# Siverteh/semantic-slam-master

Hardware: NVIDIA B200
Metric: frame-pairs/sec extract+match @640x480, 2048 kpts (higher is better)
Workload: dtype f16x3 (fp32 in/out)

## Files before the change

include/sslam_b200.h:

```cpp
#ifndef SSLAM_B200_H_
#define SSLAM_B200_H_

#include <stddef.h>
#include <stdint.h>

#ifdef __cplusplus
extern "C" {
#endif

#define SSLAM_ABI_VERSION 4

enum {
  SSLAM_OK = 0,
  SSLAM_EINVAL = -1,
  SSLAM_EUNSUPPORTED = -2,
  SSLAM_EWORKSPACE = -3,
  SSLAM_ECUDA = -4,
  SSLAM_ENODEVICE = -5,
  SSLAM_ERANGE = -6
};

enum {
  SSLAM_INFO_BRANCH = 0,
  SSLAM_INFO_NCAND = 1,
  SSLAM_INFO_TIES = 2,
  SSLAM_INFO_NLOCALMAX = 3
};

enum {
  SSLAM_SIM_F32 = 0,
  SSLAM_SIM_TF32X3 = 1,
  SSLAM_SIM_BF16 = 2,
  SSLAM_SIM_F16X3 = 3
};

enum {
  SSLAM_MATCH_M1 = 1,
  SSLAM_MATCH_M2 = 2,
  SSLAM_MATCH_M3 = 3,
  SSLAM_MATCH_M4 = 4,
  SSLAM_MATCH_M5 = 5
};

int sslam_abi_version(void);

int sslam_last_error(char* buf, size_t len);

int sslam_device_check(void);

uint64_t sslam_launch_count(void);

int sslam_profile_enable(int on);
int sslam_profile_kinds(void);
const char* sslam_profile_kind_name(int kind);
int sslam_profile_read(int kind, double* total_ms, uint64_t* launches);

size_t sslam_decode_workspace_bytes(int B, int H, int W, int K);
int sslam_decode_topk_f32(const float* sal, int from_logits, int B, int H, int W, int K,
                          int nms_radius, float pct, float floor, float* kpts_xy, float* scores,
                          int32_t* info, void* ws, size_t ws_bytes, void* stream);

int sslam_nms_f32(const float* sal, int B, int H, int W, int nms_radius, float* out, void* stream);

int sslam_gather_bilinear_f32(const float* feat, const float* kpts, int B, int h, int w, int C,
                              int N, int coords, float* out, void* out_hi, void* out_lo,
                              void* stream);

int sslam_l2norm_rows(const float* in, int rows, int D, float eps, float* out_f32,
                      void* out_bf16, void* out_hi, void* out_lo, void* stream);

size_t sslam_refiner_packed_bytes(int C, int Hd, int D, int blocks);
int sslam_refiner_pack_weights(const float* const* params, int C, int Hd, int D, int blocks,
                               void* packed, size_t packed_bytes, void* stream);
size_t sslam_refiner_workspace_bytes(int rows, int C, int Hd, int D, int blocks);
int sslam_refiner_forward_f32(const float* const* params, const void* packed, const float* x,
                              const void* x_hi, const void* x_lo,
                              int rows, int C, int Hd, int D, int blocks, float eps_norm,
                              float* out_f32, void* out_bf16, void* out_hi, void* out_lo,
                              void* ws, size_t ws_bytes, void* stream);
int sslam_refiner_range_check(void* stream);

size_t sslam_match_workspace_bytes(int F1, int F2, int P, int N, int M, int D, int dtype);
int sslam_match_top2(const void* bank1, const void* bank1_lo, int F1, const void* bank2,
                     const void* bank2_lo, int F2, const int32_t* pair_index, int dtype,
                     int P, int N, int M, int D, int32_t* nn12, float* best12, float* second12,
                     int32_t* nn21, float* best21, void* ws, size_t ws_bytes, void* stream);

int sslam_match_finalize(int variant, const double* params ,
                         const int32_t* pair_index, int P, int N, int M, const int32_t* nn12,
                         const float* best12, const float* second12, const int32_t* nn21,
                         const float* best21, const float* scores1, const float* scores2,
                         const float* inten1, const float* inten2, int32_t* pairs,
                         float* pair_scores, int32_t* counts, void* stream);

int sslam_nn_points(const float* kpts1, int F1, const float* kpts2, int F2, const double* H,
                    const int32_t* pair_index, int P, int N, int M, void* min_dist, int32_t* argmin,
                    void* stream);

int sslam_gt_matches(const void* min_dist, const int32_t* argmin, int is_double, double threshold, int P,
                     int N, int32_t* pairs, int32_t* counts, void* stream);

int sslam_eval_matches(const int32_t* pred, const int32_t* pred_counts, int pred_stride,
                       const int32_t* gt, const int32_t* gt_counts, int gt_stride, int P, int N,
                       int32_t* scratch, int32_t* out, void* stream);

size_t sslam_ransac_workspace_bytes(int P, int L, int iters);
int sslam_ransac_homography(const float* kpts1, int F1, const float* kpts2, int F2,
                            const int32_t* pair_index, int P, int N, int M,
                            const int32_t* pairs, const float* pair_scores, const int32_t* counts, int L,
                            int iters, double threshold, uint64_t seed,
                            double* H, int32_t* out_pairs, float* out_scores,
                            int32_t* out_counts, uint8_t* inlier_mask,
                            void* ws, size_t ws_bytes, void* stream);

int sslam_heatmap_from_cells_f32(const float* logits, int B, int Hc, int Wc, int cell, int border,
                                 float* heat, void* stream);

size_t sslam_selector_packed_bytes(int C, int hidden);
int sslam_selector_pack_weights(const float* conv1_weight, int C, int hidden, void* packed,
                                size_t packed_bytes, void* stream);
size_t sslam_selector_workspace_bytes(int B, int H, int W, int C);
int sslam_selector_head_f32(const float* feat, const void* packed, const float* conv1_bias,
                            const float* conv2_weight, const float* conv2_bias, int B, int H, int W,
                            int C, int hidden, int apply_sigmoid, float* out, void* ws,
                            size_t ws_bytes, void* stream);

#ifdef __cplusplus
}
#endif
#endif
```

semantic-slam-master_b200/csrc/gather.cu:

```cuda
#include <cuda_bf16.h>
#include <cuda_fp16.h>

#include "common.cuh"

namespace sslam {
namespace {

constexpr int WARPS_PER_BLOCK = 8;

struct Taps {
  int off[4];
  float w[4];
};

struct TapGeom {
  int xi0, yi0;
  bool vx0, vx1, vy0, vy1;
  float w[4];
};

__device__ __forceinline__ TapGeom tap_geometry(float x, float y, int H, int W, int coords) {
  if (coords == 1) {
    x = __fmul_rn(__fsub_rn(x, 8.0f), 0.0625f);
    y = __fmul_rn(__fsub_rn(y, 8.0f), 0.0625f);
  }
  const float wm1 = (float)(W - 1), hm1 = (float)(H - 1);
  float nx = __fsub_rn(__fdiv_rn(__fmul_rn(2.0f, x), wm1), 1.0f);
  float ny = __fsub_rn(__fdiv_rn(__fmul_rn(2.0f, y), hm1), 1.0f);
  float ix = __fmul_rn(__fmul_rn(__fadd_rn(nx, 1.0f), 0.5f), wm1);
  float iy = __fmul_rn(__fmul_rn(__fadd_rn(ny, 1.0f), 0.5f), hm1);
  float x0 = floorf(ix), y0 = floorf(iy);
  float x1 = __fadd_rn(x0, 1.0f), y1 = __fadd_rn(y0, 1.0f);
  float wx0 = __fsub_rn(x1, ix), wx1 = __fsub_rn(ix, x0);
  float wy0 = __fsub_rn(y1, iy), wy1 = __fsub_rn(iy, y0);
  TapGeom g;
  g.w[0] = __fmul_rn(wx0, wy0); g.w[1] = __fmul_rn(wx1, wy0);
  g.w[2] = __fmul_rn(wx0, wy1); g.w[3] = __fmul_rn(wx1, wy1);
  g.xi0 = (int)x0; g.yi0 = (int)y0;
  const int xi1 = (int)x1, yi1 = (int)y1;
  g.vx0 = (x0 >= 0.f) && (g.xi0 < W); g.vx1 = (x1 >= 0.f) && (xi1 < W);
  g.vy0 = (y0 >= 0.f) && (g.yi0 < H); g.vy1 = (y1 >= 0.f) && (yi1 < H);
  return g;
}

__device__ __forceinline__ Taps make_taps(float x, float y, int H, int W, int C, int coords) {
  const TapGeom g = tap_geometry(x, y, H, W, coords);
  Taps t;
#pragma unroll
  for (int i = 0; i < 4; ++i) t.w[i] = g.w[i];
  const int xi1 = g.xi0 + 1, yi1 = g.yi0 + 1;
  t.off[0] = (g.vx0 && g.vy0) ? (g.yi0 * W + g.xi0) * C : -1;
  t.off[1] = (g.vx1 && g.vy0) ? (g.yi0 * W + xi1) * C : -1;
  t.off[2] = (g.vx0 && g.vy1) ? (yi1 * W + g.xi0) * C : -1;
  t.off[3] = (g.vx1 && g.vy1) ? (yi1 * W + xi1) * C : -1;
  return t;
}

__device__ __forceinline__ float blend(float a, float b, float c, float d, const Taps& t) {
  float acc = __fmul_rn(a, t.w[0]);
  acc = __fmaf_rn(b, t.w[1], acc);
  acc = __fmaf_rn(c, t.w[2], acc);
  acc = __fmaf_rn(d, t.w[3], acc);
  return acc;
}

template <bool VEC4>
__global__ void __launch_bounds__(WARPS_PER_BLOCK * 32)
gather_kernel(const float* __restrict__ feat, const float* __restrict__ kpts, int B, int H, int W,
              int C, int N, int coords, float* __restrict__ out, __half* __restrict__ out_hi,
              __half* __restrict__ out_lo) {
  const int lane = threadIdx.x & 31;
  const long long kp = (long long)blockIdx.x * WARPS_PER_BLOCK + (threadIdx.x >> 5);
  if (kp >= (long long)B * N) return;
  const int b = (int)(kp / N);
  const float x = __ldg(kpts + 2 * kp), y = __ldg(kpts + 2 * kp + 1);
  const Taps t = make_taps(x, y, H, W, C, coords);
  const float* img = feat + (size_t)b * H * W * C;
  float* o = out + (size_t)kp * C;
  if (VEC4) {
    const float4 zero = make_float4(0.f, 0.f, 0.f, 0.f);
    for (int c = lane * 4; c < C; c += 128) {
      float4 v0 = t.off[0] >= 0 ? __ldg(reinterpret_cast<const float4*>(img + t.off[0] + c)) : zero;
      float4 v1 = t.off[1] >= 0 ? __ldg(reinterpret_cast<const float4*>(img + t.off[1] + c)) : zero;
      float4 v2 = t.off[2] >= 0 ? __ldg(reinterpret_cast<const float4*>(img + t.off[2] + c)) : zero;
      float4 v3 = t.off[3] >= 0 ? __ldg(reinterpret_cast<const float4*>(img + t.off[3] + c)) : zero;
      float4 r;
      r.x = blend(v0.x, v1.x, v2.x, v3.x, t);
      r.y = blend(v0.y, v1.y, v2.y, v3.y, t);
      r.z = blend(v0.z, v1.z, v2.z, v3.z, t);
      r.w = blend(v0.w, v1.w, v2.w, v3.w, t);
      if (out) *reinterpret_cast<float4*>(o + c) = r;
      if (out_hi) {
        __half h4[4], l4[4];
        const float rr[4] = {r.x, r.y, r.z, r.w};
#pragma unroll
        for (int i = 0; i < 4; ++i) {
          h4[i] = __float2half_rn(rr[i]);
          l4[i] = __float2half_rn(__fmul_rn(__fsub_rn(rr[i], __half2float(h4[i])), 2048.0f));
        }
        *reinterpret_cast<uint2*>(out_hi + (size_t)kp * C + c) = *reinterpret_cast<uint2*>(h4);
        *reinterpret_cast<uint2*>(out_lo + (size_t)kp * C + c) = *reinterpret_cast<uint2*>(l4);
      }
    }
  } else {
    for (int c = lane; c < C; c += 32) {
      float v0 = t.off[0] >= 0 ? __ldg(img + t.off[0] + c) : 0.f;
      float v1 = t.off[1] >= 0 ? __ldg(img + t.off[1] + c) : 0.f;
      float v2 = t.off[2] >= 0 ? __ldg(img + t.off[2] + c) : 0.f;
      float v3 = t.off[3] >= 0 ? __ldg(img + t.off[3] + c) : 0.f;
      const float r = blend(v0, v1, v2, v3, t);
      if (out) o[c] = r;
      if (out_hi) {
        const __half h = __float2half_rn(r);
        out_hi[(size_t)kp * C + c] = h;
        out_lo[(size_t)kp * C + c] = __float2half_rn(__fmul_rn(__fsub_rn(r, __half2float(h)), 2048.0f));
      }
    }
  }
}

constexpr int BAND_THREADS = 512;

__device__ __forceinline__ uint32_t smem_addr_u32(const void* p) {
  return static_cast<uint32_t>(__cvta_generic_to_shared(p));
}
__device__ __forceinline__ void band_bar_wait(uint64_t* bar, uint32_t parity) {
  const uint32_t addr = smem_addr_u32(bar);
  uint32_t ok = 0;
  while (!ok)
    asm volatile(
        "{\n"
        ".reg .pred p;\n"
        "mbarrier.try_wait.parity.shared::cta.b64 p, [%1], %2;\n"
        "selp.u32 %0, 1, 0, p;\n"
        "}\n"
        : "=r"(ok)
        : "r"(addr), "r"(parity)
        : "memory");
}

struct __align__(4) BandGeo { float w[4]; short xi0; short band; };

template <bool PAIR>
__global__ void __launch_bounds__(BAND_THREADS, 1)
gather_band_kernel(const float* __restrict__ feat, const float* __restrict__ kpts, int B, int H, int W, int C,
                   int N, int coords, float* __restrict__ out, __half* __restrict__ out_hi,
                   __half* __restrict__ out_lo, int bands_per_group, int ngroups) {
  extern __shared__ __align__(128) unsigned char gsm[];
  const int row_bytes = W * C * 4, row_floats = W * C;
  const float* ring = reinterpret_cast<const float*>(gsm);
  BandGeo* geo = reinterpret_cast<BandGeo*>(gsm + 3 * row_bytes);
  unsigned short* list = reinterpret_cast<unsigned short*>(geo + N);
  uint64_t* bars = reinterpret_cast<uint64_t*>((reinterpret_cast<uintptr_t>(list + N) + 7) & ~(uintptr_t)7);
  __shared__ int list_n[2];
  const int tid = threadIdx.x, lane = tid & 31, warp = tid >> 5;
  const int b = blockIdx.x / ngroups, g = blockIdx.x - b * ngroups;
  const int band_lo = g * bands_per_group - 1;
  const int band_hi = min(band_lo + bands_per_group, H);
  const float* img = feat + (size_t)b * H * W * C;
  const float* kp_b = kpts + (size_t)b * N * 2;

  if (tid == 0) {
    for (int i = 0; i < 3; ++i)
      asm volatile("mbarrier.init.shared::cta.b64 [%0], 1;" ::"r"(smem_addr_u32(&bars[i])) : "memory");
    asm volatile("fence.mbarrier_init.release.cluster;" ::: "memory");
    list_n[0] = 0; list_n[1] = 0;
  }
  const int first_row = max(band_lo, 0);
  const int last_row = min(band_hi, H - 1);
  __syncthreads();
  auto issue_row = [&](int y) {
    const int slot = y % 3;
    const uint32_t bar = smem_addr_u32(&bars[slot]);
    const int use = (y - first_row) / 3;
    if (use > 0) band_bar_wait(&bars[slot], (uint32_t)(use - 1) & 1u);
    asm volatile("mbarrier.arrive.expect_tx.shared::cta.b64 _, [%0], %1;" ::"r"(bar), "r"((uint32_t)row_bytes) : "memory");
    asm volatile("cp.async.bulk.shared::cluster.global.mbarrier::complete_tx::bytes [%0], [%1], %2, [%3];" ::"r"(
                     smem_addr_u32(gsm + (size_t)slot * row_bytes)),
                 "l"(img + (size_t)y * W * C), "r"((uint32_t)row_bytes), "r"(bar)
                 : "memory");
  };
  if (tid == 0) {
    if (first_row <= last_row) issue_row(first_row);
    if (first_row + 1 <= last_row) issue_row(first_row + 1);
  }
  for (int i = tid; i < N; i += BAND_THREADS) {
    const float2 xy = __ldg(reinterpret_cast<const float2*>(kp_b) + i);
    const TapGeom t = tap_geometry(xy.x, xy.y, H, W, coords);
    BandGeo gg;
#pragma unroll
    for (int k = 0; k < 4; ++k) gg.w[k] = t.w[k];
    const bool any_x = t.vx0 || t.vx1, any_y = t.vy0 || t.vy1;
    gg.xi0 = (short)((any_x && any_y) ? (t.vx0 ? t.xi0 : -1) : -2);
    gg.band = (short)((any_x && any_y && t.vy0) ? t.yi0 : -1);
    geo[i] = gg;
  }
  __syncthreads();

  int it = 0;
  for (int y0 = band_lo; y0 < band_hi; ++y0, ++it) {
    if (tid == 0 && y0 + 2 <= last_row && y0 + 2 >= first_row + 2) issue_row(y0 + 2);
    const bool r0_ok = y0 >= 0 && y0 < H, r1_ok = y0 + 1 >= 0 && y0 + 1 < H;
    const int o0 = ((y0 + 3) % 3) * row_floats, o1 = ((y0 + 1) % 3) * row_floats;
    int* cnt = &list_n[it & 1];
    for (int i = tid; i < N; i += BAND_THREADS)
      if (geo[i].band == y0) list[atomicAdd(cnt, 1)] = (unsigned short)i;
    __syncthreads();
    const int n = *cnt;
    if (tid == 0) list_n[(it + 1) & 1] = 0;
    if (r0_ok) band_bar_wait(&bars[y0 % 3], (uint32_t)((y0 - first_row) / 3) & 1u);
    if (r1_ok) band_bar_wait(&bars[(y0 + 1) % 3], (uint32_t)((y0 + 1 - first_row) / 3) & 1u);
    for (int e = warp; e < n; e += BAND_THREADS / 32) {
      const int i = list[e];
      const BandGeo gg = geo[i];
      const size_t kp = (size_t)b * N + i;
      Taps w4;
#pragma unroll
      for (int k = 0; k < 4; ++k) w4.w[k] = gg.w[k];
      const int xi0 = gg.xi0;
      const bool vx0 = xi0 >= 0 && xi0 < W, vx1 = xi0 >= -1 && xi0 + 1 < W;
      const int t0 = (vx0 && r0_ok) ? o0 + xi0 * C : -1, t1 = (vx1 && r0_ok) ? o0 + (xi0 + 1) * C : -1;
      const int t2 = (vx0 && r1_ok) ? o1 + xi0 * C : -1, t3 = (vx1 && r1_ok) ? o1 + (xi0 + 1) * C : -1;
      const float4 zero = make_float4(0.f, 0.f, 0.f, 0.f);
      for (int c = lane * 4; c < C; c += 128) {
        const float4 a0 = t0 >= 0 ? *reinterpret_cast<const float4*>(ring + t0 + c) : zero;
        const float4 a1 = t1 >= 0 ? *reinterpret_cast<const float4*>(ring + t1 + c) : zero;
        const float4 a2 = t2 >= 0 ? *reinterpret_cast<const float4*>(ring + t2 + c) : zero;
        const float4 a3 = t3 >= 0 ? *reinterpret_cast<const float4*>(ring + t3 + c) : zero;
        float4 r;
        r.x = blend(a0.x, a1.x, a2.x, a3.x, w4);
        r.y = blend(a0.y, a1.y, a2.y, a3.y, w4);
        r.z = blend(a0.z, a1.z, a2.z, a3.z, w4);
        r.w = blend(a0.w, a1.w, a2.w, a3.w, w4);
        if (!PAIR) {
          *reinterpret_cast<float4*>(out + kp * C + c) = r;
        } else {
          const __half2 h01 = __floats2half2_rn(r.x, r.y), h23 = __floats2half2_rn(r.z, r.w);
          const float2 f01 = __half22float2(h01), f23 = __half22float2(h23);
          const __half2 l01 = __floats2half2_rn(__fmul_rn(__fsub_rn(r.x, f01.x), 2048.0f),
                                                __fmul_rn(__fsub_rn(r.y, f01.y), 2048.0f));
          const __half2 l23 = __floats2half2_rn(__fmul_rn(__fsub_rn(r.z, f23.x), 2048.0f),
                                                __fmul_rn(__fsub_rn(r.w, f23.y), 2048.0f));
          uint2 hv, lv;
          hv.x = *reinterpret_cast<const unsigned*>(&h01); hv.y = *reinterpret_cast<const unsigned*>(&h23);
          lv.x = *reinterpret_cast<const unsigned*>(&l01); lv.y = *reinterpret_cast<const unsigned*>(&l23);
          *reinterpret_cast<uint2*>(out_hi + kp * C + c) = hv;
          *reinterpret_cast<uint2*>(out_lo + kp * C + c) = lv;
        }
      }
    }
    __syncthreads();
  }
}

template <bool VEC4>
__global__ void __launch_bounds__(WARPS_PER_BLOCK * 32)
l2norm_kernel(const float* __restrict__ in, int rows, int D, float eps, float* __restrict__ out_f32,
              __nv_bfloat16* __restrict__ out_bf16, __half* __restrict__ out_hi, __half* __restrict__ out_lo) {
  const int lane = threadIdx.x & 31;
  const long long row = (long long)blockIdx.x * WARPS_PER_BLOCK + (threadIdx.x >> 5);
  if (row >= rows) return;
  const float* src = in + (size_t)row * D;
  float ss = 0.f;
  if (VEC4) {
    for (int c = lane * 4; c < D; c += 128) {
      float4 v = __ldg(reinterpret_cast<const float4*>(src + c));
      ss = __fmaf_rn(v.x, v.x, ss); ss = __fmaf_rn(v.y, v.y, ss);
      ss = __fmaf_rn(v.z, v.z, ss); ss = __fmaf_rn(v.w, v.w, ss);
    }
  } else {
    for (int c = lane; c < D; c += 32) { float v = __ldg(src + c); ss = __fmaf_rn(v, v, ss); }
  }
  ss = warp_reduce_sum(ss);
  const float denom = fmaxf(sqrtf(ss), eps);
  if (VEC4) {
    for (int c = lane * 4; c < D; c += 128) {
      float4 v = __ldg(reinterpret_cast<const float4*>(src + c));
      float4 r = make_float4(__fdiv_rn(v.x, denom), __fdiv_rn(v.y, denom), __fdiv_rn(v.z, denom),
                             __fdiv_rn(v.w, denom));
      if (out_f32) *reinterpret_cast<float4*>(out_f32 + (size_t)row * D + c) = r;
      if (out_bf16) {
        __nv_bfloat162 lo = __floats2bfloat162_rn(r.x, r.y), hi = __floats2bfloat162_rn(r.z, r.w);
        uint2 pk = make_uint2(*reinterpret_cast<unsigned*>(&lo), *reinterpret_cast<unsigned*>(&hi));
        *reinterpret_cast<uint2*>(out_bf16 + (size_t)row * D + c) = pk;
      }
      if (out_hi) {
        __half h4[4], l4[4];
        const float rr[4] = {r.x, r.y, r.z, r.w};
#pragma unroll
        for (int i = 0; i < 4; ++i) {
          h4[i] = __float2half_rn(rr[i]);
          l4[i] = __float2half_rn(__fmul_rn(__fsub_rn(rr[i], __half2float(h4[i])), 2048.0f));
        }
        *reinterpret_cast<uint2*>(out_hi + (size_t)row * D + c) = *reinterpret_cast<uint2*>(h4);
        *reinterpret_cast<uint2*>(out_lo + (size_t)row * D + c) = *reinterpret_cast<uint2*>(l4);
      }
    }
  } else {
    for (int c = lane; c < D; c += 32) {
      float r = __fdiv_rn(__ldg(src + c), denom);
      if (out_f32) out_f32[(size_t)row * D + c] = r;
      if (out_bf16) out_bf16[(size_t)row * D + c] = __float2bfloat16_rn(r);
      if (out_hi) {
        const __half h = __float2half_rn(r);
        out_hi[(size_t)row * D + c] = h;
        out_lo[(size_t)row * D + c] = __float2half_rn(__fmul_rn(__fsub_rn(r, __half2float(h)), 2048.0f));
      }
    }
  }
}

}
}

using namespace sslam;

extern "C" int sslam_gather_bilinear_f32(const float* feat, const float* kpts, int B, int h, int w,
                                         int C, int N, int coords, float* out, void* out_hi_, void* out_lo_,
                                         void* stream_) {
  __half* out_hi = static_cast<__half*>(out_hi_);
  __half* out_lo = static_cast<__half*>(out_lo_);
  int rc = check_device();
  if (rc) return rc;
  cudaStream_t stream = (cudaStream_t)stream_;
  SSLAM_REQUIRE(B >= 0 && h > 0 && w > 0 && C > 0 && N >= 0, SSLAM_EINVAL, "gather: bad size");
  SSLAM_REQUIRE(coords == 0 || coords == 1, SSLAM_EINVAL, "gather: coords must be 0 or 1");
  if (B == 0 || N == 0) return SSLAM_OK;
  SSLAM_REQUIRE(feat && kpts && (out || (out_hi && out_lo)), SSLAM_EINVAL, "gather: null pointer");
  SSLAM_REQUIRE((out_hi == nullptr) == (out_lo == nullptr), SSLAM_EINVAL, "gather: pair outputs go together");
  SSLAM_REQUIRE((long long)h * w * C < (1ll << 31), SSLAM_EUNSUPPORTED, "gather: map too large");
  const long long total = (long long)B * N;
  const unsigned blocks = (unsigned)((total + WARPS_PER_BLOCK - 1) / WARPS_PER_BLOCK);
  const bool vec = (C % 4 == 0) && ((reinterpret_cast<uintptr_t>(feat) & 15) == 0) &&
                   ((reinterpret_cast<uintptr_t>(out) & 15) == 0) &&
                   ((reinterpret_cast<uintptr_t>(out_hi) & 7) == 0) && ((reinterpret_cast<uintptr_t>(out_lo) & 7) == 0);
  const size_t band_smem = 3 * (size_t)w * C * 4 + (size_t)N * (sizeof(BandGeo) + 2) + 64;
  if (vec && ((size_t)w * C * 4) % 16 == 0 && N <= 65535 && band_smem <= 227 * 1024 - 256 &&
      (reinterpret_cast<uintptr_t>(kpts) & 7) == 0 && ((out != nullptr) != (out_hi != nullptr))) {
    static DeviceOnce once;
    if (once.first_use()) {
      SSLAM_CHECK_CUDA(cudaFuncSetAttribute(gather_band_kernel<true>, cudaFuncAttributeMaxDynamicSharedMemorySize,
                                            227 * 1024 - 256));
      SSLAM_CHECK_CUDA(cudaFuncSetAttribute(gather_band_kernel<false>, cudaFuncAttributeMaxDynamicSharedMemorySize,
                                            227 * 1024 - 256));
    }
    int ngroups = (8 * num_sms() + B - 1) / B;
    if (ngroups > (h + 1) / 3) ngroups = (h + 1) / 3;
    if (ngroups < 1) ngroups = 1;
    const int per = (h + 1 + ngroups - 1) / ngroups;
    ngroups = (h + 1 + per - 1) / per;
    SSLAM_LAUNCH(KK_GATHER, stream,
                 if (out_hi)
        gather_band_kernel<true><<<(unsigned)(B * ngroups), BAND_THREADS, band_smem, stream>>>(
            feat, kpts, B, h, w, C, N, coords, out, out_hi, out_lo, per, ngroups);
      else
        gather_band_kernel<false><<<(unsigned)(B * ngroups), BAND_THREADS, band_smem, stream>>>(
            feat, kpts, B, h, w, C, N, coords, out, out_hi, out_lo, per, ngroups));
    return SSLAM_OK;
  }
  SSLAM_LAUNCH(KK_GATHER, stream,
               if (vec)
      gather_kernel<true><<<blocks, WARPS_PER_BLOCK * 32, 0, stream>>>(feat, kpts, B, h, w, C, N,
                                                                      coords, out, out_hi, out_lo);
    else
      gather_kernel<false><<<blocks, WARPS_PER_BLOCK * 32, 0, stream>>>(feat, kpts, B, h, w, C, N,
                                                                     coords, out, out_hi, out_lo));
  return SSLAM_OK;
}

extern "C" int sslam_l2norm_rows(const float* in, int rows, int D, float eps, float* out_f32,
                                 void* out_bf16, void* out_hi_, void* out_lo_, void* stream_) {
  __half* out_hi = static_cast<__half*>(out_hi_);
  __half* out_lo = static_cast<__half*>(out_lo_);
  int rc = check_device();
  if (rc) return rc;
  cudaStream_t stream = (cudaStream_t)stream_;
  SSLAM_REQUIRE(rows >= 0 && D > 0, SSLAM_EINVAL, "l2norm: bad size");
  if (rows == 0) return SSLAM_OK;
  SSLAM_REQUIRE(in && (out_f32 || out_bf16 || out_hi), SSLAM_EINVAL, "l2norm: null pointer");
  SSLAM_REQUIRE((out_hi == nullptr) == (out_lo == nullptr), SSLAM_EINVAL, "l2norm: pair outputs go together");
  const unsigned blocks = (unsigned)((rows + WARPS_PER_BLOCK - 1) / WARPS_PER_BLOCK);
  const bool vec = (D % 4 == 0) && ((reinterpret_cast<uintptr_t>(in) & 15) == 0) &&
                   (!out_f32 || (reinterpret_cast<uintptr_t>(out_f32) & 15) == 0) &&
                   (!out_bf16 || (reinterpret_cast<uintptr_t>(out_bf16) & 7) == 0) &&
                   ((reinterpret_cast<uintptr_t>(out_hi) & 7) == 0) && ((reinterpret_cast<uintptr_t>(out_lo) & 7) == 0);
  SSLAM_LAUNCH(KK_L2NORM, stream,
               if (vec)
      l2norm_kernel<true><<<blocks, WARPS_PER_BLOCK * 32, 0, stream>>>(
          in, rows, D, eps, out_f32, reinterpret_cast<__nv_bfloat16*>(out_bf16), out_hi, out_lo);
    else
      l2norm_kernel<false><<<blocks, WARPS_PER_BLOCK * 32, 0, stream>>>(
          in, rows, D, eps, out_f32, reinterpret_cast<__nv_bfloat16*>(out_bf16), out_hi, out_lo));
  return SSLAM_OK;
}
```

semantic-slam-master_b200/csrc/match_f32.cu:

```cuda
#include "common.cuh"

namespace sslam {
namespace {

constexpr int BM = 128, BN = 128, BK = 16;
constexpr int LDS_ = BM + 4;
constexpr int THREADS = 256;
constexpr int MAX_D = 256;

struct Top2 {
  float best, second;
  int idx;
  __device__ __forceinline__ void init() {
    best = __int_as_float(0xff800000); second = best; idx = 0x7fffffff;
  }
  __device__ __forceinline__ void push(float v, int i) {
    if (v > best) { second = best; best = v; idx = i; }
    else second = fmaxf(second, v);
  }
  __device__ __forceinline__ void merge(float b2, float s2, int i2) {
    if (b2 > best || (b2 == best && i2 < idx)) { second = fmaxf(best, s2); best = b2; idx = i2; }
    else second = fmaxf(second, b2);
  }
};

struct MatchParams {
  const float* bank1;
  const float* bank2;
  const int32_t* pair_index;
  int P, N, M, D;
  int32_t* nn12;
  float* best12;
  float* second12;
  u64* colkeys;
};

__device__ __forceinline__ int row_of(int t, int i) { return (i < 4) ? t * 4 + i : 64 + t * 4 + (i - 4); }

__global__ void __launch_bounds__(THREADS, 1) match_f32_kernel(MatchParams p) {
  extern __shared__ __align__(16) float smem[];
  const int D = p.D, N = p.N, M = p.M;
  const int dpad = (D + BK - 1) / BK * BK;
  float* As = smem;
  float* Bs = As + (size_t)dpad * LDS_;
  u64* colpart = reinterpret_cast<u64*>(Bs + 2 * BK * LDS_);

  const int pair = blockIdx.y;
  int ia = pair, ib = pair;
  if (p.pair_index) { ia = p.pair_index[2 * pair]; ib = p.pair_index[2 * pair + 1]; }
  const float* A = p.bank1 + (size_t)ia * N * D;
  const float* Bm = p.bank2 + (size_t)ib * M * D;
  const int row0 = blockIdx.x * BM;
  const int tid = threadIdx.x, tx = tid & 15, ty = tid >> 4, lane = tid & 31, warp = tid >> 5;

  const int dq = dpad / 4;
  for (int e = tid; e < BM * dq; e += THREADS) {
    int r = e / dq, kq = e - r * dq;
    float4 v = make_float4(0.f, 0.f, 0.f, 0.f);
    if (row0 + r < N && kq * 4 < D) v = __ldg(reinterpret_cast<const float4*>(A + (size_t)(row0 + r) * D + kq * 4));
    As[(kq * 4 + 0) * LDS_ + r] = v.x; As[(kq * 4 + 1) * LDS_ + r] = v.y;
    As[(kq * 4 + 2) * LDS_ + r] = v.z; As[(kq * 4 + 3) * LDS_ + r] = v.w;
  }

  const int nkb = dpad / BK;
  const int ntile = (M + BN - 1) / BN;
  const int total = nkb * ntile;

  float4 stage[2];
  auto fetch = [&](int it) {
    int ct = it / nkb, kb = it - ct * nkb;
#pragma unroll
    for (int j = 0; j < 2; ++j) {
      int e = tid + THREADS * j, col = e >> 2, kq = e & 3;
      int gc = ct * BN + col, gk = kb * BK + kq * 4;
      stage[j] = (gc < M && gk < D) ? __ldg(reinterpret_cast<const float4*>(Bm + (size_t)gc * D + gk))
                                    : make_float4(0.f, 0.f, 0.f, 0.f);
    }
  };
  auto commit = [&](int buf) {
    float* dst = Bs + buf * BK * LDS_;
#pragma unroll
    for (int j = 0; j < 2; ++j) {
      int e = tid + THREADS * j, col = e >> 2, kq = e & 3;
      dst[(kq * 4 + 0) * LDS_ + col] = stage[j].x; dst[(kq * 4 + 1) * LDS_ + col] = stage[j].y;
      dst[(kq * 4 + 2) * LDS_ + col] = stage[j].z; dst[(kq * 4 + 3) * LDS_ + col] = stage[j].w;
    }
  };

  Top2 rowtop[8];
#pragma unroll
  for (int i = 0; i < 8; ++i) rowtop[i].init();
  float acc[8][8];
#pragma unroll
  for (int i = 0; i < 8; ++i)
#pragma unroll
    for (int j = 0; j < 8; ++j) acc[i][j] = 0.f;

  fetch(0);
  commit(0);
  __syncthreads();

  for (int it = 0; it < total; ++it) {
    const int buf = it & 1;
    const int ct = it / nkb, kb = it - ct * nkb;
    if (it + 1 < total) fetch(it + 1);
    const float* a_base = As + (size_t)(kb * BK) * LDS_;
    const float* b_base = Bs + buf * BK * LDS_;
#pragma unroll
    for (int kk = 0; kk < BK; ++kk) {
      float4 a0 = *reinterpret_cast<const float4*>(a_base + kk * LDS_ + ty * 4);
      float4 a1 = *reinterpret_cast<const float4*>(a_base + kk * LDS_ + 64 + ty * 4);
      float4 b0 = *reinterpret_cast<const float4*>(b_base + kk * LDS_ + tx * 4);
      float4 b1 = *reinterpret_cast<const float4*>(b_base + kk * LDS_ + 64 + tx * 4);
      float a[8] = {a0.x, a0.y, a0.z, a0.w, a1.x, a1.y, a1.z, a1.w};
      float b[8] = {b0.x, b0.y, b0.z, b0.w, b1.x, b1.y, b1.z, b1.w};
#pragma unroll
      for (int i = 0; i < 8; ++i)
#pragma unroll
        for (int j = 0; j < 8; ++j) acc[i][j] = __fmaf_rn(a[i], b[j], acc[i][j]);
    }
    if (kb == nkb - 1) {
      const int c0 = ct * BN;
#pragma unroll
      for (int i = 0; i < 8; ++i) {
        Top2 t; t.init();
#pragma unroll
        for (int j = 0; j < 8; ++j) {
          int gc = c0 + row_of(tx, j);
          if (gc < M) t.push(acc[i][j], gc);
        }
#pragma unroll
        for (int o = 8; o > 0; o >>= 1) {
          float b2 = __shfl_xor_sync(0xffffffffu, t.best, o);
          float s2 = __shfl_xor_sync(0xffffffffu, t.second, o);
          int i2 = __shfl_xor_sync(0xffffffffu, t.idx, o);
          t.merge(b2, s2, i2);
        }
        rowtop[i].merge(t.best, t.second, t.idx);
      }
#pragma unroll
      for (int j = 0; j < 8; ++j) {
        u64 key = 0;
        float bv = 0.f; int bi = -1;
#pragma unroll
        for (int i = 0; i < 8; ++i) {
          int gr = row0 + row_of(ty, i);
          if (gr < N && (bi < 0 || acc[i][j] > bv)) { bv = acc[i][j]; bi = gr; }
        }
        if (bi >= 0) key = pack_key(bv, (u32)bi);
        u64 other = __shfl_xor_sync(0xffffffffu, key, 16);
        key = other > key ? other : key;
        if (lane < 16) colpart[warp * BN + row_of(tx, j)] = key;
      }
      __syncthreads();
      if (tid < BN) {
        u64 k = colpart[tid];
#pragma unroll
        for (int w = 1; w < 8; ++w) { u64 o = colpart[w * BN + tid]; k = o > k ? o : k; }
        if (c0 + tid < M && k) atomicMax(p.colkeys + (size_t)pair * M + c0 + tid, k);
      }
#pragma unroll
      for (int i = 0; i < 8; ++i)
#pragma unroll
        for (int j = 0; j < 8; ++j) acc[i][j] = 0.f;
    }
    if (it + 1 < total) commit(buf ^ 1);
    __syncthreads();
  }

  if (tx == 0) {
#pragma unroll
    for (int i = 0; i < 8; ++i) {
      int gr = row0 + row_of(ty, i);
      if (gr < N) {
        size_t o = (size_t)pair * N + gr;
        p.nn12[o] = rowtop[i].idx;
        p.best12[o] = rowtop[i].best;
        p.second12[o] = rowtop[i].second;
      }
    }
  }
}

__global__ void unpack_cols_kernel(const u64* __restrict__ keys, long long total, int32_t* nn21,
                                   float* best21) {
  long long i = (long long)blockIdx.x * blockDim.x + threadIdx.x;
  if (i >= total) return;
  u64 k = keys[i];
  nn21[i] = (int32_t)key_index(k);
  best21[i] = key_value(k);
}

struct FinalizeParams {
  int variant;
  float prm[8];
  double prm_d[2];
  const int32_t* pair_index;
  int P, N, M;
  const int32_t* nn12; const float* best12; const float* second12;
  const int32_t* nn21; const float* best21;
  const float* scores1; const float* scores2; const float* inten1; const float* inten2;
  int32_t* pairs; float* pair_scores; int32_t* counts;
};

__device__ __forceinline__ bool accept_row(const FinalizeParams& f, int pair, int ia, int ib, int i,
                                           int& j, float& score) {
  const size_t ro = (size_t)pair * f.N + i;
  j = f.nn12[ro];
  const float best = f.best12[ro];
  const bool mutual = (f.nn21[(size_t)pair * f.M + j] == i);
  switch (f.variant) {
    case SSLAM_MATCH_M1: {
      float second = fmaxf(f.second12[ro], -1.0f);
      score = best;
      if (f.prm[1] != 0.f) return mutual && ((double)best > __dmul_rn((double)second, f.prm_d[0]));
      return mutual && (best > __fmul_rn(second, f.prm[0]));
    }
    case SSLAM_MATCH_M2: {
      float s1 = f.scores1[(size_t)ia * f.N + i], s2 = f.scores2[(size_t)ib * f.M + j];
      float avg = __fdiv_rn(__fadd_rn(s1, s2), 2.0f);
      bool ok = mutual && (avg >= f.prm[1]) && (best >= f.prm[2]);
      if (f.inten1 && f.inten2) {
        float a = f.inten1[(size_t)ia * f.N + i], b = f.inten2[(size_t)ib * f.M + j];
        ok = ok && (__fdiv_rn(__fadd_rn(a, b), 2.0f) >= f.prm[3]);
      }
      score = __fadd_rn(__fmul_rn(f.prm[4], best), __fmul_rn(f.prm[0], avg));
      return ok;
    }
    case SSLAM_MATCH_M3: {
      float ratio = __fdiv_rn(f.second12[ro], __fadd_rn(best, 1e-8f));
      score = __fsub_rn(1.0f, best);
      return mutual && (ratio < f.prm[0]);
    }
    case SSLAM_MATCH_M4:
      score = best;
      return mutual;
    default:
      score = best;
      return best > f.prm[0];
  }
}

__global__ void __launch_bounds__(256) finalize_kernel(FinalizeParams f) {
  __shared__ int scan[256];
  __shared__ int total_s;
  const int pair = blockIdx.x, tid = threadIdx.x;
  int ia = pair, ib = pair;
  if (f.pair_index) { ia = f.pair_index[2 * pair]; ib = f.pair_index[2 * pair + 1]; }
  const int seg = (f.N + 255) / 256;
  const int beg = min(f.N, tid * seg), end = min(f.N, beg + seg);
  int cnt = 0;
  for (int i = beg; i < end; ++i) { int j; float s; cnt += accept_row(f, pair, ia, ib, i, j, s) ? 1 : 0; }
  scan[tid] = cnt;
  __syncthreads();
  for (int o = 1; o < 256; o <<= 1) {
    int v = (tid >= o) ? scan[tid - o] : 0;
    __syncthreads();
    scan[tid] += v;
    __syncthreads();
  }
  int pos = scan[tid] - cnt;
  if (tid == 255) total_s = scan[255];
  __syncthreads();
  const int total = total_s;
  int32_t* pr = f.pairs + (size_t)pair * f.N * 2;
  float* ps = f.pair_scores + (size_t)pair * f.N;
  for (int i = beg; i < end; ++i) {
    int j; float s;
    if (accept_row(f, pair, ia, ib, i, j, s)) { pr[2 * pos] = i; pr[2 * pos + 1] = j; ps[pos] = s; ++pos; }
  }
  for (int i = total + tid; i < f.N; i += 256) { pr[2 * i] = -1; pr[2 * i + 1] = -1; ps[i] = 0.f; }
  if (tid == 0) f.counts[pair] = total;
}

}

int match_top2_tc(const void* bank1, const void* bank1_lo, int F1, const void* bank2, const void* bank2_lo,
                  int F2, const int32_t* pair_index,
                  int dtype, int P, int N, int M, int D, int32_t* nn12, float* best12, float* second12,
                  u64* colkeys, void* ws_extra, size_t ws_extra_bytes, cudaStream_t stream);
size_t match_tc_extra_workspace(int P, int N, int M, int D, int dtype, int F1, int F2);

}

using namespace sslam;

extern "C" size_t sslam_match_workspace_bytes(int F1, int F2, int P, int N, int M, int D, int dtype) {
  if (P <= 0 || N <= 0 || M <= 0) return 0;
  size_t base = align_up((size_t)P * M * sizeof(u64), 256);
  if (dtype != SSLAM_SIM_F32) base += match_tc_extra_workspace(P, N, M, D, dtype, F1, F2);
  return base;
}

extern "C" int sslam_match_top2(const void* bank1, const void* bank1_lo, int F1, const void* bank2,
                                const void* bank2_lo, int F2, const int32_t* pair_index,
                                int dtype, int P, int N, int M, int D, int32_t* nn12, float* best12,
                                float* second12, int32_t* nn21, float* best21, void* ws,
                                size_t ws_bytes, void* stream_) {
  int rc = check_device();
  if (rc) return rc;
  cudaStream_t stream = (cudaStream_t)stream_;
  SSLAM_REQUIRE(P >= 0 && N >= 0 && M >= 0 && D > 0, SSLAM_EINVAL, "match: bad size");
  if (P == 0 || N == 0) return SSLAM_OK;
  SSLAM_REQUIRE(M > 0, SSLAM_EINVAL, "match: M must be > 0 (argmax of an empty row)");
  SSLAM_REQUIRE(bank1 && bank2 && nn12 && best12 && second12 && nn21 && best21 && ws, SSLAM_EINVAL,
                "match: null pointer");
  SSLAM_REQUIRE(D % 4 == 0 && D <= MAX_D, SSLAM_EUNSUPPORTED, "match: D=%d (need D%%4==0, D<=256)", D);
  SSLAM_REQUIRE(dtype == SSLAM_SIM_F32 || dtype == SSLAM_SIM_TF32X3 || dtype == SSLAM_SIM_BF16 ||
                    dtype == SSLAM_SIM_F16X3,
                SSLAM_EINVAL, "match: unknown dtype %d", dtype);
  SSLAM_REQUIRE(F1 > 0 && F2 > 0 && (pair_index || (F1 >= P && F2 >= P)), SSLAM_EINVAL,
                "match: banks hold %d / %d sets but %d implicit pairs were requested", F1, F2, P);
  const bool presplit = bank1_lo != nullptr || bank2_lo != nullptr;
  SSLAM_REQUIRE(!presplit || (dtype == SSLAM_SIM_F16X3 && bank1_lo && bank2_lo), SSLAM_EINVAL,
                "match: pre-split banks need SSLAM_SIM_F16X3 and both lo arrays");
  {
    const size_t need = presplit ? align_up((size_t)P * M * sizeof(u64), 256)
                                 : sslam_match_workspace_bytes(F1, F2, P, N, M, D, dtype);
    SSLAM_REQUIRE(ws_bytes >= need, SSLAM_EWORKSPACE, "match: workspace %zu < %zu", ws_bytes, need);
  }
  SSLAM_REQUIRE((reinterpret_cast<uintptr_t>(bank1) & 15) == 0 &&
                (reinterpret_cast<uintptr_t>(bank2) & 15) == 0, SSLAM_EINVAL,
                "match: descriptor banks must be 16-byte aligned");
  u64* colkeys = reinterpret_cast<u64*>(ws);
  const size_t colbytes = align_up((size_t)P * M * sizeof(u64), 256);
  SSLAM_CHECK_CUDA(cudaMemsetAsync(colkeys, 0, (size_t)P * M * sizeof(u64), stream));

  if (dtype == SSLAM_SIM_F32) {
    MatchParams mp;
    mp.bank1 = (const float*)bank1; mp.bank2 = (const float*)bank2; mp.pair_index = pair_index;
    mp.P = P; mp.N = N; mp.M = M; mp.D = D;
    mp.nn12 = nn12; mp.best12 = best12; mp.second12 = second12; mp.colkeys = colkeys;
    const int dpad = (D + BK - 1) / BK * BK;
    size_t smem = ((size_t)dpad * LDS_ + 2 * BK * LDS_) * 4 + 8 * BN * sizeof(u64);
    static DeviceOnce once;
    if (once.first_use()) {
      SSLAM_CHECK_CUDA(cudaFuncSetAttribute(match_f32_kernel,
                                            cudaFuncAttributeMaxDynamicSharedMemorySize, 200 * 1024));
    }
    dim3 grid((N + BM - 1) / BM, P);
    SSLAM_LAUNCH(KK_MATCH_F32, stream,
                 match_f32_kernel<<<grid, THREADS, smem, stream>>>(mp));
  } else {
    rc = match_top2_tc(bank1, bank1_lo, F1, bank2, bank2_lo, F2, pair_index, dtype, P, N, M, D, nn12, best12,
                       second12, colkeys,
                       reinterpret_cast<char*>(ws) + colbytes, ws_bytes - colbytes, stream);
    if (rc) return rc;
  }
  const long long total = (long long)P * M;
  SSLAM_LAUNCH(KK_UNPACK, stream,
               unpack_cols_kernel<<<(unsigned)((total + 255) / 256), 256, 0, stream>>>(colkeys, total, nn21, best21));
  return SSLAM_OK;
}

extern "C" int sslam_match_finalize(int variant, const double* params, const int32_t* pair_index,
                                    int P, int N, int M, const int32_t* nn12, const float* best12,
                                    const float* second12, const int32_t* nn21, const float* best21,
                                    const float* scores1, const float* scores2, const float* inten1,
                                    const float* inten2, int32_t* pairs, float* pair_scores,
                                    int32_t* counts, void* stream_) {
  int rc = check_device();
  if (rc) return rc;
  cudaStream_t stream = (cudaStream_t)stream_;
  SSLAM_REQUIRE(variant >= SSLAM_MATCH_M1 && variant <= SSLAM_MATCH_M5, SSLAM_EINVAL,
                "finalize: unknown variant %d", variant);
  SSLAM_REQUIRE(P >= 0 && N >= 0 && M > 0, SSLAM_EINVAL, "finalize: bad size");
  if (P == 0) return SSLAM_OK;
  SSLAM_REQUIRE(params && nn12 && best12 && second12 && nn21 && best21 && pairs && pair_scores && counts,
                SSLAM_EINVAL, "finalize: null pointer");
  SSLAM_REQUIRE(variant != SSLAM_MATCH_M2 || (scores1 && scores2), SSLAM_EINVAL,
                "finalize: M2 needs saliency scores");
  FinalizeParams f;
  f.variant = variant;
  for (int i = 0; i < 8; ++i) f.prm[i] = (float)params[i];
  f.prm_d[0] = params[0]; f.prm_d[1] = params[1];
  f.pair_index = pair_index; f.P = P; f.N = N; f.M = M;
  f.nn12 = nn12; f.best12 = best12; f.second12 = second12; f.nn21 = nn21; f.best21 = best21;
  f.scores1 = scores1; f.scores2 = scores2; f.inten1 = inten1; f.inten2 = inten2;
  f.pairs = pairs; f.pair_scores = pair_scores; f.counts = counts;
  SSLAM_LAUNCH(KK_FINALIZE, stream,
               finalize_kernel<<<P, 256, 0, stream>>>(f));
  return SSLAM_OK;
}
```

semantic-slam-master_b200/csrc/match_tc.cu:

```cuda
#include "tc_common.cuh"

#include <mutex>

namespace sslam {

using namespace tc;

long long* g_match_dbg = nullptr;

namespace {

constexpr int BM = 128, BN = 128;
constexpr int BLOCK_BYTES = BM * 128;
constexpr int NUM_THREADS = 192;
constexpr int TP_LD = 36;

template <int MODE> struct Cfg;
template <> struct Cfg<SSLAM_SIM_TF32X3> {
  static constexpr int TERMS = 2, STAGES = 3, BK = 32, ACC_COLS = 2 * BN, TMEM_COLS = 512;
  static constexpr bool TF32 = true;
  static constexpr uint32_t FMT = FMT_TF32;
  static constexpr float CROSS_SCALE = 1.0f;
};
struct TcParams {
// ... 351 lines not shown
          tcgen05_fence_after();
          const uint32_t tmem_d = tmem_base + acc * C::ACC_COLS;
          for (int kb = 0; kb < nkb; ++kb) {
            if (dbg_on) tq = clock64();
            if (ct == 0) mbar_wait(&afull[kb], (uint32_t)(it & 1));
            if (dbg_on) w_afull += clock64() - tq;
            if (dbg_on) tq = clock64();
            mbar_wait(&full[stage], phase);
            if (dbg_on) w_full += clock64() - tq;
            tcgen05_fence_after();
            const uint32_t sa = smem_u32(a_res + (kb * C::TERMS) * BLOCK_BYTES);
            const uint32_t sb = smem_u32(b_stages + stage * L::B_STAGE);
            const uint64_t a_hi = make_smem_desc_sw128(sa);
            const uint64_t a_lo = make_smem_desc_sw128(sa + BLOCK_BYTES);
            const uint64_t b_hi = make_smem_desc_sw128(sb);
            const uint64_t b_lo = make_smem_desc_sw128(sb + L::B_TILE);
#pragma unroll
            for (int k = 0; k < 4; ++k) {
              const uint64_t adv = (uint64_t)(k * 32 >> 4);
              const uint32_t first = (kb | k) ? 1u : 0u;
              if (C::TERMS == 2) {
                umma_ss_pair(tmem_d + BN, a_lo + adv, b_hi + adv, idesc, first);
                umma_ss_pair(tmem_d + BN, a_hi + adv, b_lo + adv, idesc, 1u);
              }
              umma_ss_pair(tmem_d, a_hi + adv, b_hi + adv, idesc, first);
            }
            tcgen05_commit_pair(&empty[stage], 3);
            if (ct == ntile - 1) tcgen05_commit_pair(&aempty[kb], 3);
            if (kb == nkb - 1) tcgen05_commit_pair(&tfull[acc], 3);
            if (++stage == C::B_STAGES) { stage = 0; phase ^= 1; }
          }
        }
      }
      if (p.dbg) {
        long long* d = p.dbg + 4 * blockIdx.x;
        d[0] = clock64() - t_begin; d[1] = w_full; d[2] = w_tempty; d[3] = w_afull;
      }
    }
  } else {
    const int q = warp & 3;
    const int ew = warp - 2;
    const int half = ew >> 2;
    const int et = threadIdx.x - 64;
    float* tp = transp + ew * 32 * R_UNIT;
    const int sc = lane & 15, srh = lane >> 4;
    const float NEG_INF = __int_as_float(0xff800000);
    int tc = 0, it = 0;
    const uint32_t tempty_leader0 = mapa_u32(smem_u32(&tempty[0]), 0);
    const uint32_t tempty_leader1 = mapa_u32(smem_u32(&tempty[1]), 0);
    for (int item = pair_id; item < nitems; item += npairs, ++it) {
      const int pair = item / strips2;
      const int row0 = (2 * (item - pair * strips2) + (int)rank) * BM;
      const int grow = row0 + q * 32 + lane;
      const bool row_ok = grow < p.N;
      int nvalid = p.N - (row0 + q * 32);
      nvalid = nvalid < 0 ? 0 : (nvalid > 32 ? 32 : nvalid);
      float best = NEG_INF, second = NEG_INF;
      int bidx = 0x7fffffff;
      for (int ct = 0; ct < ntile; ++ct, ++tc) {
        const int acc = tc & 1;
        mbar_wait(&tfull[acc], ((uint32_t)tc >> 1) & 1u);
        tcgen05_fence_after();
        u64* cp = colpart + (acc * 4 + q) * BN;
        const int c0 = ct * BN;
        uint32_t r[R_UNIT], rs[R_UNIT];
        {
          const uint32_t taddr = tmem_base + ((uint32_t)(q * 32) << 16) + acc * C::ACC_COLS + half * 64;
          tmem_ld_32x16(taddr, r);
          if (C::TERMS == 2) tmem_ld_32x16(taddr + BN, rs);
        }
#pragma unroll
        for (int un = 0; un < 64 / R_UNIT; ++un) {
          const int col0 = half * 64 + un * R_UNIT;
          const int gc0 = c0 + col0;
          float v[R_UNIT];
          tmem_ld_wait();
#pragma unroll
          for (int j = 0; j < R_UNIT; ++j)
            v[j] = C::TERMS == 2 ? __fmaf_rn(__uint_as_float(rs[j]), C::CROSS_SCALE, __uint_as_float(r[j]))
                                 : __uint_as_float(r[j]);
          if (un + 1 < 64 / R_UNIT) {
            const uint32_t taddr = tmem_base + ((uint32_t)(q * 32) << 16) + acc * C::ACC_COLS + col0 + R_UNIT;
            tmem_ld_32x16(taddr, r);
            if (C::TERMS == 2) tmem_ld_32x16(taddr + BN, rs);
          }
          if (gc0 + R_UNIT > p.M) {
#pragma unroll
            for (int j = 0; j < R_UNIT; ++j)
              if (gc0 + j >= p.M) v[j] = NEG_INF;
          }
          {
            float tb[R_UNIT / 2], ts[R_UNIT / 2];
#pragma unroll
            for (int j = 0; j < R_UNIT / 2; ++j) {
              tb[j] = fmaxf(v[2 * j], v[2 * j + 1]);
              ts[j] = fminf(v[2 * j], v[2 * j + 1]);
            }
#pragma unroll
            for (int w = R_UNIT / 4; w >= 1; w >>= 1) {
#pragma unroll
              for (int j = 0; j < w; ++j) {
                const float lo = fminf(tb[2 * j], tb[2 * j + 1]);
                ts[j] = fmaxf(fmaxf(ts[2 * j], ts[2 * j + 1]), lo);
                tb[j] = fmaxf(tb[2 * j], tb[2 * j + 1]);
              }
            }
            const float ub = tb[0];
            second = fmaxf(fmaxf(second, ts[0]), fminf(best, ub));
            if (ub > best) {
              best = ub;
              int f = R_UNIT - 1;
#pragma unroll
              for (int j = R_UNIT - 2; j >= 0; --j) f = (v[j] == ub) ? j : f;
              bidx = gc0 + f;
            }
          }
          if (nvalid < 32 && !row_ok) {
#pragma unroll
            for (int j = 0; j < R_UNIT; ++j) v[j] = NEG_INF;
          }
          __syncwarp();
#pragma unroll
          for (int j = 0; j < R_UNIT / 4; ++j)
            *reinterpret_cast<float4*>(tp + lane * R_UNIT + ((j ^ ((lane >> 1) & 3)) << 2)) =
                make_float4(v[4 * j], v[4 * j + 1], v[4 * j + 2], v[4 * j + 3]);
          __syncwarp();
          float cv[16];
#pragma unroll
          for (int rr = 0; rr < 16; ++rr)
            cv[rr] = tp[(2 * rr + srh) * R_UNIT + ((((sc >> 2) ^ (rr & 3))) << 2) + (sc & 3)];
          float m0 = cv[0], m1 = cv[8];
          int r0 = 0, r1 = 8;
#pragma unroll
          for (int rr = 1; rr < 8; ++rr) {
            if (cv[rr] > m0) { m0 = cv[rr]; r0 = rr; }
            if (cv[8 + rr] > m1) { m1 = cv[8 + rr]; r1 = 8 + rr; }
          }
          float cm = m0;
          int cr = r0;
          if (m1 > m0) { cm = m1; cr = r1; }
          cr = 2 * cr + srh;
          {
            const float om = __shfl_xor_sync(0xffffffffu, cm, 16);
            const int orow = __shfl_xor_sync(0xffffffffu, cr, 16);
            if (om > cm || (om == cm && orow < cr)) { cm = om; cr = orow; }
          }
          if (srh == 0) cp[col0 + sc] = (nvalid > 0) ? pack_key(cm, (u32)(row0 + q * 32 + cr)) : 0ull;
        }
        tcgen05_fence_before();
        __syncwarp();
        if (lane == 0) mbar_arrive_cluster(acc ? tempty_leader1 : tempty_leader0);
        named_bar_sync(1, 32 * R_EPI_WARPS);
        if (et < BN) {
          const u64* base = colpart + acc * 4 * BN;
          u64 k = base[et];
#pragma unroll
          for (int w = 1; w < 4; ++w) { u64 o = base[w * BN + et]; k = o > k ? o : k; }
          if (c0 + et < p.M && k) atomicMax(p.colkeys + (size_t)pair * p.M + c0 + et, k);
        }
      }
      float* rm = rowmerge + (it & 1) * (BM * 3) + (q * 32 + lane) * 3;
      if (half == 1) { rm[0] = best; rm[1] = __int_as_float(bidx); rm[2] = second; }
      named_bar_sync(1, 32 * R_EPI_WARPS);
      if (half == 0 && row_ok) {
        const float ob = rm[0], os = rm[2];
        const int oi = __float_as_int(rm[1]);
        const float lo_best = fminf(best, ob);
        float sec = fmaxf(fmaxf(second, os), lo_best);
        if (ob > best || (ob == best && oi < bidx)) { best = ob; bidx = oi; }
        const size_t o = (size_t)pair * p.N + grow;
        p.nn12[o] = bidx; p.best12[o] = best; p.second12[o] = sec;
      }
    }
  }
  tcgen05_fence_before();
  cluster_sync_all();
  if (warp == 1) tmem_dealloc_pair(tmem_base, C::TMEM_COLS);
}

__global__ void split_tf32_kernel(const float4* __restrict__ src, float4* __restrict__ hi,
                                  float4* __restrict__ lo, size_t n4) {
  size_t i = (size_t)blockIdx.x * blockDim.x + threadIdx.x;
  const size_t stride = (size_t)gridDim.x * blockDim.x;
  for (; i < n4; i += stride) {
    float4 x = __ldg(src + i), h, l;
    h.x = to_tf32_rna(x.x); h.y = to_tf32_rna(x.y); h.z = to_tf32_rna(x.z); h.w = to_tf32_rna(x.w);
    l.x = to_tf32_rna(__fsub_rn(x.x, h.x)); l.y = to_tf32_rna(__fsub_rn(x.y, h.y));
    l.z = to_tf32_rna(__fsub_rn(x.z, h.z)); l.w = to_tf32_rna(__fsub_rn(x.w, h.w));
    hi[i] = h; lo[i] = l;
  }
}

__global__ void split_f16_kernel(const float4* __restrict__ src, uint2* __restrict__ hi,
                                 uint2* __restrict__ lo, size_t n4) {
  size_t i = (size_t)blockIdx.x * blockDim.x + threadIdx.x;
  const size_t stride = (size_t)gridDim.x * blockDim.x;
  for (; i < n4; i += stride) {
    const float4 x = __ldg(src + i);
    __half h[4], l[4];
    split_f16(x.x, h[0], l[0]); split_f16(x.y, h[1], l[1]);
    split_f16(x.z, h[2], l[2]); split_f16(x.w, h[3], l[3]);
    hi[i] = *reinterpret_cast<uint2*>(h);
    lo[i] = *reinterpret_cast<uint2*>(l);
  }
}

typedef CUresult (*EncodeTiledFn)(CUtensorMap*, CUtensorMapDataType, cuuint32_t, void*, const cuuint64_t*,
                                  const cuuint64_t*, const cuuint32_t*, const cuuint32_t*,
                                  CUtensorMapInterleave, CUtensorMapSwizzle, CUtensorMapL2promotion,
                                  CUtensorMapFloatOOBfill);
EncodeTiledFn g_encode = nullptr;
std::once_flag g_encode_once;

}

namespace tc {
int make_tensor_map_2d(CUtensorMap* map, const void* base, uint64_t rows, uint64_t cols,
                       uint32_t box_rows, uint32_t box_cols, int elem_bytes, int swizzle_bytes) {
  std::call_once(g_encode_once, [] {
    void* fn = nullptr;
    cudaDriverEntryPointQueryResult qres;
    if (cudaGetDriverEntryPoint("cuTensorMapEncodeTiled", &fn, cudaEnableDefault, &qres) == cudaSuccess &&
        qres == cudaDriverEntryPointSuccess)
      g_encode = reinterpret_cast<EncodeTiledFn>(fn);
  });
  SSLAM_REQUIRE(g_encode != nullptr, SSLAM_ECUDA, "cuTensorMapEncodeTiled entry point not available");
  if (swizzle_bytes < 0) return SSLAM_OK;
  cuuint64_t dims[2] = {cols, rows};
  cuuint64_t strides[1] = {cols * (uint64_t)elem_bytes};
  cuuint32_t box[2] = {box_cols, box_rows};
  cuuint32_t estr[2] = {1, 1};
  CUresult r = g_encode(map, elem_bytes == 2 ? CU_TENSOR_MAP_DATA_TYPE_BFLOAT16 : CU_TENSOR_MAP_DATA_TYPE_FLOAT32,
                        2, const_cast<void*>(base), dims, strides, box, estr, CU_TENSOR_MAP_INTERLEAVE_NONE,
                        swizzle_bytes == 128 ? CU_TENSOR_MAP_SWIZZLE_128B
                                             : swizzle_bytes == 64 ? CU_TENSOR_MAP_SWIZZLE_64B : CU_TENSOR_MAP_SWIZZLE_NONE,
                        CU_TENSOR_MAP_L2_PROMOTION_L2_256B,
                        CU_TENSOR_MAP_FLOAT_OOB_FILL_NONE);
  SSLAM_REQUIRE(r == CUDA_SUCCESS, SSLAM_ECUDA, "cuTensorMapEncodeTiled failed with CUresult %d", (int)r);
  return SSLAM_OK;
}
int make_tensor_map_nhwc(CUtensorMap* map, const void* base, uint64_t B, uint64_t H, uint64_t W, uint64_t C,
                         uint32_t box_h, uint32_t box_w, uint32_t box_c) {
  int rc = make_tensor_map_2d(nullptr, nullptr, 0, 0, 0, 0, 0, -1);
  if (rc) return rc;
  cuuint64_t dims[4] = {C, W, H, B};
  cuuint64_t strides[3] = {C * 2, W * C * 2, H * W * C * 2};
  cuuint32_t box[4] = {box_c, box_w, box_h, 1};
  cuuint32_t estr[4] = {1, 1, 1, 1};
  CUresult r = g_encode(map, CU_TENSOR_MAP_DATA_TYPE_BFLOAT16, 4, const_cast<void*>(base), dims, strides, box, estr,
                        CU_TENSOR_MAP_INTERLEAVE_NONE, CU_TENSOR_MAP_SWIZZLE_128B, CU_TENSOR_MAP_L2_PROMOTION_L2_256B,
                        CU_TENSOR_MAP_FLOAT_OOB_FILL_NONE);
  SSLAM_REQUIRE(r == CUDA_SUCCESS, SSLAM_ECUDA, "cuTensorMapEncodeTiled (NHWC) failed with CUresult %d", (int)r);
  return SSLAM_OK;
}
}

namespace {

struct BankPlan {
  bool shared;
  size_t frames_a, frames_b, off_b_frames;
};

BankPlan plan_banks(const float* b1, int F1, const float* b2, int F2, int N, int M, int D) {
  BankPlan pl{false, (size_t)F1, (size_t)F2, 0};
  if (N != M) return pl;
  const size_t frame = (size_t)N * D;
  const float* end1 = b1 + (size_t)F1 * frame;
  if (b2 >= b1 && b2 <= end1 && ((size_t)(b2 - b1) % frame) == 0) {
    pl.shared = true;
    pl.off_b_frames = (size_t)(b2 - b1) / frame;
    size_t uni = pl.off_b_frames + (size_t)F2;
    pl.frames_a = uni > (size_t)F1 ? uni : (size_t)F1;
  }
  return pl;
}

}

size_t match_tc_extra_workspace(int P, int N, int M, int D, int dtype, int F1, int F2) {
  (void)P;
  if (dtype != SSLAM_SIM_TF32X3 && dtype != SSLAM_SIM_F16X3) return 0;
  const size_t e = dtype == SSLAM_SIM_F16X3 ? 2 : 4;
  return 2 * align_up((size_t)F1 * N * D * e, 256) + 2 * align_up((size_t)F2 * M * D * e, 256) + 1024;
}

template <int MODE>
static int launch_tc(const CUtensorMap& a_hi, const CUtensorMap& a_lo, const CUtensorMap& b_hi,
                     const CUtensorMap& b_lo, const TcParams& tp, cudaStream_t stream) {
  using L = SmemLayout<MODE>;
  static DeviceOnce once;
  if (once.first_use()) {
    SSLAM_CHECK_CUDA(cudaFuncSetAttribute(match_tc_kernel<MODE>, cudaFuncAttributeMaxDynamicSharedMemorySize,
                                          L::TOTAL));
  }
  const int strips = (tp.N + BM - 1) / BM;
  SSLAM_LAUNCH(KK_MATCH_TC, stream,
               match_tc_kernel<MODE><<<strips * tp.P, NUM_THREADS, L::TOTAL, stream>>>(a_hi, a_lo, b_hi, b_lo, tp));
  return SSLAM_OK;
}

template <int MODE>
static int launch_res(const CUtensorMap& a_hi, const CUtensorMap& a_lo, const CUtensorMap& b_hi,
                      const CUtensorMap& b_lo, const TcParams& tp, cudaStream_t stream) {
  using L = RSmem<MODE>;
  static DeviceOnce once;
  if (once.first_use()) {
    SSLAM_CHECK_CUDA(cudaFuncSetAttribute(match_res_kernel<MODE>, cudaFuncAttributeMaxDynamicSharedMemorySize,
                                          L::TOTAL));
  }
  const int items = ((((tp.N + BM - 1) / BM) + 1) / 2) * tp.P;
  const int pairs = items < num_sms() / 2 ? items : num_sms() / 2;
  const int grid = 2 * pairs;
  SSLAM_LAUNCH(KK_MATCH_TC, stream,
               match_res_kernel<MODE><<<grid, R_THREADS, L::TOTAL, stream>>>(a_hi, a_lo, b_hi, b_lo, tp));
  return SSLAM_OK;
}

int match_top2_tc(const void* bank1, const void* bank1_lo, int F1, const void* bank2, const void* bank2_lo,
                  int F2, const int32_t* pair_index,
                  int dtype, int P, int N, int M, int D, int32_t* nn12, float* best12, float* second12,
                  u64* colkeys, void* ws_extra, size_t ws_extra_bytes, cudaStream_t stream) {
  TcParams tp;
  tp.dbg = g_match_dbg;
  tp.pair_index = pair_index; tp.P = P; tp.N = N; tp.M = M; tp.D = D;
  tp.nn12 = nn12; tp.best12 = best12; tp.second12 = second12; tp.colkeys = colkeys;
  CUtensorMap a_hi, a_lo, b_hi, b_lo;
  int rc;
  if (dtype == SSLAM_SIM_BF16) {
    SSLAM_REQUIRE(D % 8 == 0, SSLAM_EUNSUPPORTED, "match(bf16): D=%d must be a multiple of 8", D);
    if ((rc = make_tensor_map_2d(&a_hi, bank1, (uint64_t)F1 * N, D, BM, 64, 2))) return rc;
    if ((rc = make_tensor_map_2d(&b_hi, bank2, (uint64_t)F2 * M, D, BN / 2, 64, 2))) return rc;
    a_lo = a_hi; b_lo = b_hi;
    return launch_res<SSLAM_SIM_BF16>(a_hi, a_lo, b_hi, b_lo, tp, stream);
  }
  const bool f16 = (dtype == SSLAM_SIM_F16X3);
  const size_t e = f16 ? 2 : 4;
  SSLAM_REQUIRE(!f16 || D % 8 == 0, SSLAM_EUNSUPPORTED, "match(f16x3): D=%d must be a multiple of 8", D);
  if (f16 && bank1_lo && bank2_lo) {
    const uint64_t rows2p = (uint64_t)F2 * M;
    if ((rc = make_tensor_map_2d(&a_hi, bank1, (uint64_t)F1 * N, D, BM, 64, 2))) return rc;
    if ((rc = make_tensor_map_2d(&a_lo, bank1_lo, (uint64_t)F1 * N, D, BM, 64, 2))) return rc;
    if ((rc = make_tensor_map_2d(&b_hi, bank2, rows2p, D, BN / 2, 64, 2))) return rc;
    if ((rc = make_tensor_map_2d(&b_lo, bank2_lo, rows2p, D, BN / 2, 64, 2))) return rc;
    return launch_res<SSLAM_SIM_F16X3>(a_hi, a_lo, b_hi, b_lo, tp, stream);
  }
  SSLAM_REQUIRE(ws_extra_bytes >= match_tc_extra_workspace(P, N, M, D, dtype, F1, F2), SSLAM_EWORKSPACE,
                "match(split): workspace too small");
  const float* f1 = static_cast<const float*>(bank1);
  const float* f2 = static_cast<const float*>(bank2);
  char* w = reinterpret_cast<char*>((reinterpret_cast<uintptr_t>(ws_extra) + 1023) & ~(uintptr_t)1023);
  const BankPlan pl = plan_banks(f1, F1, f2, F2, N, M, D);
  const size_t n1 = pl.frames_a * (size_t)N * D;
  char* h1 = w;
  char* l1 = w + align_up(n1 * e, 256);
  const int sms = num_sms();
  auto split = [&](const float* src, char* hi, char* lo, size_t n) -> int {
    if (f16)
      SSLAM_LAUNCH(KK_SPLIT, stream,
                   split_f16_kernel<<<sms * 8, 256, 0, stream>>>(reinterpret_cast<const float4*>(src),
                                                                 reinterpret_cast<uint2*>(hi),
                                                                 reinterpret_cast<uint2*>(lo), n / 4));
    else
      SSLAM_LAUNCH(KK_SPLIT, stream,
                   split_tf32_kernel<<<sms * 8, 256, 0, stream>>>(reinterpret_cast<const float4*>(src),
                                                                  reinterpret_cast<float4*>(hi),
                                                                  reinterpret_cast<float4*>(lo), n / 4));
    return SSLAM_OK;
  };
  if ((rc = split(f1, h1, l1, n1))) return rc;
  char *h2, *l2;
  if (pl.shared) {
    h2 = h1 + pl.off_b_frames * (size_t)N * D * e;
    l2 = l1 + pl.off_b_frames * (size_t)N * D * e;
  } else {
    const size_t n2 = (size_t)F2 * M * D;
    char* w2 = w + 2 * align_up(n1 * e, 256);
    h2 = w2;
    l2 = w2 + align_up(n2 * e, 256);
    if ((rc = split(f2, h2, l2, n2))) return rc;
  }
  const uint64_t rows2 = (uint64_t)F2 * M;
  if (f16) {
    if ((rc = make_tensor_map_2d(&a_hi, h1, (uint64_t)F1 * N, D, BM, 64, 2))) return rc;
    if ((rc = make_tensor_map_2d(&a_lo, l1, (uint64_t)F1 * N, D, BM, 64, 2))) return rc;
    if ((rc = make_tensor_map_2d(&b_hi, h2, rows2, D, BN / 2, 64, 2))) return rc;
    if ((rc = make_tensor_map_2d(&b_lo, l2, rows2, D, BN / 2, 64, 2))) return rc;
    return launch_res<SSLAM_SIM_F16X3>(a_hi, a_lo, b_hi, b_lo, tp, stream);
  }
  if ((rc = make_tensor_map_2d(&a_hi, h1, (uint64_t)F1 * N, D, BM, 32, 4))) return rc;
  if ((rc = make_tensor_map_2d(&a_lo, l1, (uint64_t)F1 * N, D, BM, 32, 4))) return rc;
  if ((rc = make_tensor_map_2d(&b_hi, h2, rows2, D, BN, 32, 4))) return rc;
  if ((rc = make_tensor_map_2d(&b_lo, l2, rows2, D, BN, 32, 4))) return rc;
  return launch_tc<SSLAM_SIM_TF32X3>(a_hi, a_lo, b_hi, b_lo, tp, stream);
}

}

extern "C" void sslam_debug_match_stalls(long long* buf) { sslam::g_match_dbg = buf; }
```

semantic-slam-master_b200/csrc/refiner_tc.cu:

```cuda
#include "tc_common.cuh"

namespace sslam {

using namespace tc;

__device__ unsigned int g_refiner_status = 0;
constexpr float F16_RANGE_SQ = 65504.0f * 65504.0f;

long long* g_gemm_dbg = nullptr;
int g_refiner_fused = 3;

namespace {

constexpr int BM = 128, BN = 128, BK = 64;
constexpr int BLOCK_BYTES = BM * 128;
constexpr int STAGES = 3;
constexpr int STAGE_BYTES = 4 * BLOCK_BYTES;
constexpr int EPI_WARPS = 8;
constexpr int NUM_THREADS = 64 + 32 * EPI_WARPS;
constexpr int TMEM_COLS = 512;
constexpr int UNIT = 16;
constexpr int STG_BYTES = 32 * UNIT * 4;
constexpr int SMEM_OPERANDS = STAGES * STAGE_BYTES;
constexpr int SMEM_TRANSP = EPI_WARPS * STG_BYTES;
// ... 1213 lines not shown
            __syncwarp();
            if (lane == 0) mbar_arrive(&tdone[tcn & 3u]);
            ++tcn;
          }
        }
      }
    }
#ifdef SSLAM_FUSED_SECTIONS
    if (c.dbg_wait && warp == 2) {
      long long* d = p.dbg + 16 * blockIdx.x + 6;
      d[0] = clock64() - t_begin;
      for (int i = 0; i < 8; ++i) d[1 + i] = sec[i];
    }
#endif
  }
  tcgen05_fence_before();
  cluster_sync_all();
  if (warp == 1) tmem_dealloc_pair(tmem_base, TMEM_COLS);
}

__global__ void split_kernel(const float4* __restrict__ src, uint2* __restrict__ hi, uint2* __restrict__ lo,
                             size_t n4) {
  size_t i = (size_t)blockIdx.x * blockDim.x + threadIdx.x;
  const size_t stride = (size_t)gridDim.x * blockDim.x;
  for (; i < n4; i += stride) {
    const float4 x = __ldg(src + i);
    __half h[4], l[4];
    split_f16(x.x, h[0], l[0]); split_f16(x.y, h[1], l[1]);
    split_f16(x.z, h[2], l[2]); split_f16(x.w, h[3], l[3]);
    hi[i] = *reinterpret_cast<uint2*>(h);
    lo[i] = *reinterpret_cast<uint2*>(l);
  }
}

__global__ void fold_ln_kernel(const float* __restrict__ W, const float* __restrict__ gamma,
                               const float* __restrict__ beta, const float* __restrict__ bias, int N, int K,
                               __half* __restrict__ hi, __half* __restrict__ lo, float* __restrict__ s1,
                               float* __restrict__ c0) {
  const int lane = threadIdx.x & 31;
  const int n = blockIdx.x * (blockDim.x >> 5) + (threadIdx.x >> 5);
  if (n >= N) return;
  float a = 0.f, c = 0.f;
  for (int k = lane; k < K; k += 32) {
    const float w = W[(size_t)n * K + k];
    const float wp = __fmul_rn(w, gamma[k]);
    __half h, l;
    split_f16(wp, h, l);
    hi[(size_t)n * K + k] = h;
    lo[(size_t)n * K + k] = l;
    a += join_f16(h, l);
    c = __fmaf_rn(beta[k], w, c);
  }
  a = warp_reduce_sum(a);
  c = warp_reduce_sum(c);
  if (lane == 0) { s1[n] = a; c0[n] = c + bias[n]; }
}

struct Pair { __half* hi; __half* lo; };

int launch_split(const float* src, Pair dst, size_t n, cudaStream_t stream) {
  SSLAM_LAUNCH(KK_SPLIT, stream,
               split_kernel<<<num_sms() * 8, 256, 0, stream>>>(reinterpret_cast<const float4*>(src),
                                                               reinterpret_cast<uint2*>(dst.hi),
                                                               reinterpret_cast<uint2*>(dst.lo), n / 4));
  return SSLAM_OK;
}

struct RowStats { float* sum; float* sq; int parts; };

size_t stat_stride_of(int rows) { return align_up((size_t)rows, 64); }
int stat_parts_of(int N) { return (N + BN - 1) / BN; }

int launch_gemm(Pair a, Pair w, int rows, int N, int K, const float* bias, RowStats a_ln, const float* s1,
                Pair residual, int relu, float* out_f32, Pair out, RowStats* out_stats, cudaStream_t stream) {
  const bool pair = (K + BK - 1) / BK <= P_MAX_KB && (N + BN - 1) / BN <= 4;
  CUtensorMap ta_hi, ta_lo, tb_hi, tb_lo;
  int rc;
  if ((rc = make_tensor_map_2d(&ta_hi, a.hi, rows, K, BM, BK, 2))) return rc;
  if ((rc = make_tensor_map_2d(&ta_lo, a.lo, rows, K, BM, BK, 2))) return rc;
  if ((rc = make_tensor_map_2d(&tb_hi, w.hi, N, K, pair ? 64 : BN, BK, 2))) return rc;
  if ((rc = make_tensor_map_2d(&tb_lo, w.lo, N, K, pair ? 64 : BN, BK, 2))) return rc;
  CUtensorMap to_hi, to_lo, to_f32;
  if (out.hi) {
    if ((rc = make_tensor_map_2d(&to_hi, out.hi, rows, N, 32, UNIT, 2, 0))) return rc;
    if ((rc = make_tensor_map_2d(&to_lo, out.lo, rows, N, 32, UNIT, 2, 0))) return rc;
    to_f32 = to_hi;
  } else {
    if ((rc = make_tensor_map_2d(&to_f32, out_f32, rows, N, 32, UNIT, 4, 0))) return rc;
    to_hi = to_f32; to_lo = to_f32;
  }
  static DeviceOnce once;
  if (once.first_use()) {
    SSLAM_CHECK_CUDA(cudaFuncSetAttribute(gemm_f16x3_kernel, cudaFuncAttributeMaxDynamicSharedMemorySize,
                                          SMEM_TOTAL));
  }
  GemmParams gp;
  gp.rows = rows; gp.N = N; gp.K = K; gp.bias = bias; gp.res_hi = residual.hi; gp.res_lo = residual.lo;
  gp.relu = relu; gp.out_f32 = out_f32; gp.out_hi = out.hi; gp.out_lo = out.lo;
  gp.a_sum = a_ln.sum; gp.a_sq = a_ln.sq; gp.a_parts = a_ln.parts; gp.s1 = s1;
  gp.out_sum = out_stats ? out_stats->sum : nullptr;
  gp.out_sq = out_stats ? out_stats->sq : nullptr;
  gp.stat_stride = stat_stride_of(rows);
  gp.dbg = g_gemm_dbg;
  if (pair) {
    const int ntile = (N + BN - 1) / BN;
    const int nsp = (rows + 2 * BM - 1) / (2 * BM);
    int groups = 0;
    if (out_stats) out_stats->parts = ntile;
    const bool ln = a_ln.sum != nullptr, res = residual.hi != nullptr, st = out_stats != nullptr;
#define SSLAM_PAIR_LAUNCH(LN_, RES_, RELU_, F32_, ST_)                                                     \
  do {                                                                                                     \
    auto kfn = gemm_pair_kernel<LN_, RES_, RELU_, F32_, ST_>;                                              \
    static std::atomic<int> max_clusters[64][5] = {};              \
    int dev_ = 0;                                                                                          \
    SSLAM_CHECK_CUDA(cudaGetDevice(&dev_));                                                                \
    dev_ &= 63;                                                                                            \
    cudaLaunchConfig_t cfg = {};                                                                           \
    cudaLaunchAttribute attr[1];                                                                           \
    attr[0].id = cudaLaunchAttributeClusterDimension;                                                      \
    attr[0].val.clusterDim.x = 2 * ntile; attr[0].val.clusterDim.y = 1; attr[0].val.clusterDim.z = 1;      \
    cfg.blockDim = dim3(NUM_THREADS); cfg.dynamicSmemBytes = P_SMEM_TOTAL; cfg.stream = stream;            \
    cfg.attrs = attr; cfg.numAttrs = 1;                                                                    \
    int mcl = max_clusters[dev_][ntile].load();                                                               \
    if (mcl == 0) {                                                                                        \
      SSLAM_CHECK_CUDA(cudaFuncSetAttribute(kfn, cudaFuncAttributeMaxDynamicSharedMemorySize, P_SMEM_TOTAL)); \
      cfg.gridDim = dim3(2 * ntile);                                                                       \
      SSLAM_CHECK_CUDA(cudaOccupancyMaxActiveClusters(&mcl, kfn, &cfg));                                   \
      SSLAM_REQUIRE(mcl >= 1, SSLAM_EUNSUPPORTED, "refiner: no cluster of %d CTAs fits on this device", 2 * ntile); \
      max_clusters[dev_][ntile].store(mcl);                                                                \
    }                                                                                                      \
    groups = mcl < nsp ? mcl : nsp;                                           \
    cfg.gridDim = dim3(2u * ntile * groups);                                                               \
    SSLAM_LAUNCH(KK_GEMM, stream,                                                                          \
                 cudaLaunchKernelEx(&cfg, kfn, ta_hi, ta_lo, tb_hi, tb_lo, to_hi, to_lo, to_f32, gp, groups)); \
  } while (0)
    if (!ln && !res && relu && !out_f32 && st) SSLAM_PAIR_LAUNCH(false, false, true, false, true);
    else if (!ln && !res && relu && !out_f32 && !st) SSLAM_PAIR_LAUNCH(false, false, true, false, false);
    else if (ln && !res && relu && !out_f32 && st) SSLAM_PAIR_LAUNCH(true, false, true, false, true);
    else if (ln && res && relu && !out_f32 && st) SSLAM_PAIR_LAUNCH(true, true, true, false, true);
    else if (ln && res && relu && !out_f32 && !st) SSLAM_PAIR_LAUNCH(true, true, true, false, false);
    else if (!ln && !res && !relu && out_f32 && !st) SSLAM_PAIR_LAUNCH(false, false, false, true, false);
    else SSLAM_REQUIRE(false, SSLAM_EUNSUPPORTED, "refiner: layer option combination not instantiated");
#undef SSLAM_PAIR_LAUNCH
    return SSLAM_OK;
  }
  if (out_stats) out_stats->parts = 1;
  const int strips = (rows + BM - 1) / BM;
  const int grid = strips < num_sms() ? strips : num_sms();
  SSLAM_LAUNCH(KK_GEMM, stream,
               gemm_f16x3_kernel<<<grid, NUM_THREADS, SMEM_TOTAL, stream>>>(ta_hi, ta_lo, tb_hi, tb_lo, to_hi, to_lo,
                                                                            to_f32, gp));
  return SSLAM_OK;
}

bool fused_eligible(int C, int Hd, int D, int blocks) {
  const int nt = (Hd + BN - 1) / BN;
  return g_refiner_fused > 0 && C <= P_MAX_KB * BK && Hd <= P_MAX_KB * BK && D <= nt * BN &&
         2 + 2 * blocks <= F_MAX_LAYERS;
}
size_t fused_scratch_rows(int rows, int Hd) {
  const size_t nt = (size_t)(Hd + BN - 1) / BN;
  const size_t nsp = ((size_t)rows + 2 * BM - 1) / (2 * BM);
  const size_t cap = 160 / (2 * nt);
  return (nsp < cap ? nsp : cap) * F_MAX_SLOTS * 2 * BM;
}
size_t fused_scratch_bytes(int rows, int Hd) {
  const size_t r = fused_scratch_rows(rows, Hd), nt = (size_t)(Hd + BN - 1) / BN;
  const size_t hd_pad = (size_t)(Hd + F_BK - 1) / F_BK * F_BK;
  return 2 * 2 * align_up(r * hd_pad * 2, 1024) + 4 * align_up(2 * nt * r * 4, 256) + 2048;
}

struct FusedLayer { Pair w; const float* bias; const float* s1; };

int launch_fused(Pair xs, const FusedLayer* layers, int rows, int C, int Hd, int D, int blocks, float* raw,
                 char* scratch, cudaStream_t stream) {
  const int L = 2 + 2 * blocks;
  const int ntile = (Hd + BN - 1) / BN;
  const int nsp = (rows + 2 * BM - 1) / (2 * BM);
  static std::atomic<int> max_clusters[64][5] = {};
  int dev = 0;
  SSLAM_CHECK_CUDA(cudaGetDevice(&dev));
  dev &= 63;
  cudaLaunchConfig_t cfg = {};
  cudaLaunchAttribute attr[1];
  attr[0].id = cudaLaunchAttributeClusterDimension;
  attr[0].val.clusterDim.x = 2 * ntile; attr[0].val.clusterDim.y = 1; attr[0].val.clusterDim.z = 1;
  cfg.blockDim = dim3(F_THREADS); cfg.dynamicSmemBytes = F_SMEM_TOTAL; cfg.stream = stream;
  cfg.attrs = attr; cfg.numAttrs = 1;
  int mcl = max_clusters[dev][ntile].load();
  if (mcl == 0) {
    SSLAM_CHECK_CUDA(cudaFuncSetAttribute(refiner_fused_kernel, cudaFuncAttributeMaxDynamicSharedMemorySize, F_SMEM_TOTAL));
    cfg.gridDim = dim3(2 * ntile);
    SSLAM_CHECK_CUDA(cudaOccupancyMaxActiveClusters(&mcl, refiner_fused_kernel, &cfg));
    SSLAM_REQUIRE(mcl >= 1, SSLAM_EUNSUPPORTED, "refiner: no cluster of %d CTAs fits on this device", 2 * ntile);
    max_clusters[dev][ntile].store(mcl);
  }
  int groups = mcl < nsp ? mcl : nsp;
  const int cap = 160 / (2 * ntile);
  if (groups > cap) groups = cap;
  int S = g_refiner_fused & 255;
  if (S > F_MAX_SLOTS) S = F_MAX_SLOTS;
  const int per_cluster = (nsp + groups - 1) / groups;
  if (S > per_cluster) S = per_cluster;
  const size_t srows = (size_t)groups * S * 2 * BM;
  SSLAM_REQUIRE(srows <= fused_scratch_rows(rows, Hd), SSLAM_EWORKSPACE, "refiner: fused scratch too small");

  const size_t hd_pad = (size_t)(Hd + F_BK - 1) / F_BK * F_BK;
  char* wp = reinterpret_cast<char*>(align_up(reinterpret_cast<uintptr_t>(scratch), 1024));
  auto take = [&](size_t bytes, size_t al) { char* q = wp; wp += align_up(bytes, al); return q; };
  Pair sh{reinterpret_cast<__half*>(take(srows * hd_pad * 4, 1024)), nullptr};
  sh.lo = sh.hi + SCR_PART;
  Pair su{reinterpret_cast<__half*>(take(srows * hd_pad * 4, 1024)), nullptr};
  su.lo = su.hi + SCR_PART;
  if (hd_pad != (size_t)Hd)
    SSLAM_CHECK_CUDA(cudaMemsetAsync(sh.hi, 0, 2 * align_up(srows * hd_pad * 4, 1024), stream));
  FusedParams fp = {};
  for (int i = 0; i < 2; ++i) {
    fp.st_sum[i] = reinterpret_cast<float*>(take((size_t)2 * ntile * srows * 4, 256));
    fp.st_sq[i] = reinterpret_cast<float*>(take((size_t)2 * ntile * srows * 4, 256));
  }
  fp.rows = rows; fp.C = C; fp.Hd = Hd; fp.D = D; fp.L = L; fp.S = S; fp.groups = groups; fp.ntile = ntile;
  fp.s_hi[0] = sh.hi; fp.s_lo[0] = sh.lo; fp.s_hi[1] = su.hi; fp.s_lo[1] = su.lo; fp.raw = raw; fp.stat_stride = srows;
  fp.dbg = g_gemm_dbg;
  fp.dbg_flags = g_refiner_fused >> 8;

  FusedMaps m;
  int rc;
  if ((rc = make_tensor_map_2d(&m.a_hi[0], xs.hi, rows, C, BM, F_BK, 2, 128))) return rc;
  if ((rc = make_tensor_map_2d(&m.a_lo[0], xs.lo, rows, C, BM, F_BK, 2, 128))) return rc;
  const uint64_t flat_rows = srows * hd_pad * 4 / 1024;
  if ((rc = make_tensor_map_2d(&m.a_hi[1], sh.hi, flat_rows, 256, F_STAGE_BYTES / 1024, 256, 4, 0))) return rc;
  if ((rc = make_tensor_map_2d(&m.a_hi[2], su.hi, flat_rows, 256, F_STAGE_BYTES / 1024, 256, 4, 0))) return rc;
  m.a_lo[1] = m.a_hi[1]; m.a_lo[2] = m.a_hi[2];
  for (int l = 0; l < F_MAX_LAYERS; ++l) {
    const int ll = l < L ? l : L - 1;
    const int K = ll == 0 ? C : Hd, N = ll == L - 1 ? D : Hd;
    if ((rc = make_tensor_map_2d(&m.w_hi[l], layers[ll].w.hi, N, K, 64, BK, 2))) return rc;
    if ((rc = make_tensor_map_2d(&m.w_lo[l], layers[ll].w.lo, N, K, 64, BK, 2))) return rc;
    fp.bias[l] = layers[ll].bias;
    fp.s1[l] = layers[ll].s1;
  }
  cfg.gridDim = dim3(2u * ntile * groups);
  SSLAM_LAUNCH(KK_GEMM, stream, cudaLaunchKernelEx(&cfg, refiner_fused_kernel, m, fp));
  return SSLAM_OK;
}

size_t pair_bytes(size_t n) { return 2 * align_up(n * 2, 256); }
size_t vec_bytes(size_t n) { return 2 * align_up(n * 4, 256); }
size_t packed_total(int C, int Hd, int D, int blocks) {
  return pair_bytes((size_t)Hd * C) + (size_t)blocks * 2 * (pair_bytes((size_t)Hd * Hd) + vec_bytes(Hd)) +
         pair_bytes((size_t)D * Hd);
}

}
}

using namespace sslam;

extern "C" size_t sslam_refiner_packed_bytes(int C, int Hd, int D, int blocks) {
  if (C <= 0 || Hd <= 0 || D <= 0 || blocks < 0) return 0;
  return packed_total(C, Hd, D, blocks) + 256;
}

extern "C" int sslam_refiner_pack_weights(const float* const* params, int C, int Hd, int D, int blocks,
                                          void* packed, size_t packed_bytes, void* stream_) {
  int rc = check_device();
  if (rc) return rc;
  cudaStream_t stream = (cudaStream_t)stream_;
  SSLAM_REQUIRE(params && packed, SSLAM_EINVAL, "refiner_pack: null pointer");
  SSLAM_REQUIRE(C % 8 == 0 && Hd % 8 == 0 && D % 4 == 0, SSLAM_EUNSUPPORTED,
                "refiner: C and hidden must be multiples of 8, D of 4 (C=%d Hd=%d D=%d)", C, Hd, D);
  SSLAM_REQUIRE(packed_bytes >= sslam_refiner_packed_bytes(C, Hd, D, blocks), SSLAM_EWORKSPACE,
                "refiner_pack: packed buffer too small");
  char* w = static_cast<char*>(packed);
  auto take_pair = [&](size_t n) {
    Pair d{reinterpret_cast<__half*>(w), reinterpret_cast<__half*>(w + align_up(n * 2, 256))};
    w += pair_bytes(n);
    return d;
  };
  if ((rc = launch_split(params[0], take_pair((size_t)Hd * C), (size_t)Hd * C, stream))) return rc;
  for (int b = 0; b < blocks; ++b) {
    const float* const* bp = params + 2 + 8 * b;
    for (int half = 0; half < 2; ++half) {
      Pair d = take_pair((size_t)Hd * Hd);
      float* s1 = reinterpret_cast<float*>(w);
      float* c0 = reinterpret_cast<float*>(w + align_up((size_t)Hd * 4, 256));
      w += vec_bytes(Hd);
      SSLAM_LAUNCH(KK_SPLIT, stream,
                   fold_ln_kernel<<<(Hd + 7) / 8, 256, 0, stream>>>(bp[4 * half + 2], bp[4 * half], bp[4 * half + 1],
                                                                    bp[4 * half + 3], Hd, Hd, d.hi, d.lo, s1, c0));
    }
  }
  return launch_split(params[2 + 8 * blocks], take_pair((size_t)D * Hd), (size_t)D * Hd, stream);
}

extern "C" size_t sslam_refiner_workspace_bytes(int rows, int C, int Hd, int D, int blocks) {
  (void)blocks;
  if (rows <= 0) return 0;
  const size_t r = (size_t)rows;
  return (r * C + 3 * r * Hd + r * D) * 4 + 6 * (size_t)stat_parts_of(Hd) * stat_stride_of(rows) * 4 + 16 * 256 +
         fused_scratch_bytes(rows, Hd);
}

extern "C" int sslam_refiner_forward_f32(const float* const* params, const void* packed, const float* x,
                                         const void* x_hi, const void* x_lo,
                                         int rows, int C, int Hd, int D, int blocks, float eps_norm,
                                         float* out_f32, void* out_bf16, void* out_hi, void* out_lo,
                                         void* ws, size_t ws_bytes, void* stream_) {
  int rc = check_device();
  if (rc) return rc;
  cudaStream_t stream = (cudaStream_t)stream_;
  SSLAM_REQUIRE(rows >= 0, SSLAM_EINVAL, "refiner: negative rows");
  if (rows == 0) return SSLAM_OK;
  SSLAM_REQUIRE(params && packed && (x || (x_hi && x_lo)) && ws && (out_f32 || out_bf16 || out_hi), SSLAM_EINVAL,
                "refiner: null pointer");
  SSLAM_REQUIRE(C % 8 == 0 && Hd % 8 == 0 && D % 4 == 0 && Hd <= MAX_N && D <= MAX_N, SSLAM_EUNSUPPORTED,
                "refiner: C and hidden must be multiples of 8, D of 4, hidden and D <= 1024 (C=%d Hd=%d D=%d)", C, Hd, D);
  SSLAM_REQUIRE(!x || (reinterpret_cast<uintptr_t>(x) & 15) == 0, SSLAM_EINVAL, "refiner: x must be 16-byte aligned");
  SSLAM_REQUIRE(ws_bytes >= sslam_refiner_workspace_bytes(rows, C, Hd, D, blocks), SSLAM_EWORKSPACE,
                "refiner: workspace %zu < %zu", ws_bytes, sslam_refiner_workspace_bytes(rows, C, Hd, D, blocks));
  const size_t r = (size_t)rows;
  char* wp = static_cast<char*>(ws);
  auto take_pair = [&](size_t n) {
    Pair q{reinterpret_cast<__half*>(wp), reinterpret_cast<__half*>(wp + align_up(n * 2, 256))};
    wp += pair_bytes(n);
    return q;
  };
  auto take_stats = [&]() {
    const size_t n = (size_t)stat_parts_of(Hd) * stat_stride_of(rows);
    RowStats st{reinterpret_cast<float*>(wp), reinterpret_cast<float*>(wp) + n, 0};
    wp += 2 * n * 4;
    return st;
  };
  Pair xs = take_pair(r * C), h_a = take_pair(r * Hd), h_b = take_pair(r * Hd), u = take_pair(r * Hd);
  RowStats st_a = take_stats(), st_b = take_stats(), st_u = take_stats();
  float* raw = reinterpret_cast<float*>(wp);
  char* fused_scratch = reinterpret_cast<char*>(align_up(reinterpret_cast<uintptr_t>(wp) + r * D * 4, 256));
  const char* pk = static_cast<const char*>(packed);
  auto next_w = [&](size_t n) {
    Pair q{reinterpret_cast<__half*>(const_cast<char*>(pk)),
           reinterpret_cast<__half*>(const_cast<char*>(pk) + align_up(n * 2, 256))};
    pk += pair_bytes(n);
    return q;
  };
  const Pair none{nullptr, nullptr};
  const RowStats no_stats{nullptr, nullptr, 0};

  if (x) {
    if ((rc = launch_split(x, xs, r * C, stream))) return rc;
  } else {
    xs.hi = static_cast<__half*>(const_cast<void*>(x_hi));
    xs.lo = static_cast<__half*>(const_cast<void*>(x_lo));
  }
  if (fused_eligible(C, Hd, D, blocks)) {
    FusedLayer layers[F_MAX_LAYERS];
    int nl = 0;
    layers[nl++] = FusedLayer{next_w((size_t)Hd * C), params[1], nullptr};
    for (int b = 0; b < blocks; ++b)
      for (int half = 0; half < 2; ++half) {
        const Pair wl = next_w((size_t)Hd * Hd);
        const float* s1 = reinterpret_cast<const float*>(pk);
        const float* c0 = reinterpret_cast<const float*>(pk + align_up((size_t)Hd * 4, 256));
        pk += vec_bytes(Hd);
        layers[nl++] = FusedLayer{wl, c0, s1};
      }
    layers[nl++] = FusedLayer{next_w((size_t)D * Hd), params[3 + 8 * blocks], nullptr};
    if ((rc = launch_fused(xs, layers, rows, C, Hd, D, blocks, raw, fused_scratch, stream))) return rc;
    return sslam_l2norm_rows(raw, rows, D, eps_norm, out_f32, out_bf16, out_hi, out_lo, stream_);
  }
  Pair w = next_w((size_t)Hd * C);
  if ((rc = launch_gemm(xs, w, rows, Hd, C, params[1], no_stats, nullptr, none, 1, nullptr, h_a,
                        blocks ? &st_a : nullptr, stream)))
    return rc;
  Pair h_cur = h_a, h_nxt = h_b;
  RowStats st_cur = st_a, st_nxt = st_b;
  for (int b = 0; b < blocks; ++b) {
    w = next_w((size_t)Hd * Hd);
    const float* s1 = reinterpret_cast<const float*>(pk);
    const float* c0 = reinterpret_cast<const float*>(pk + align_up((size_t)Hd * 4, 256));
    pk += vec_bytes(Hd);
    if ((rc = launch_gemm(h_cur, w, rows, Hd, Hd, c0, st_cur, s1, none, 1, nullptr, u, &st_u, stream))) return rc;
    w = next_w((size_t)Hd * Hd);
    s1 = reinterpret_cast<const float*>(pk);
    c0 = reinterpret_cast<const float*>(pk + align_up((size_t)Hd * 4, 256));
    pk += vec_bytes(Hd);
    const bool last = (b == blocks - 1);
    if ((rc = launch_gemm(u, w, rows, Hd, Hd, c0, st_u, s1, h_cur, 1, nullptr, h_nxt, last ? nullptr : &st_nxt,
                          stream)))
      return rc;
    Pair tp = h_cur; h_cur = h_nxt; h_nxt = tp;
    RowStats ts = st_cur; st_cur = st_nxt; st_nxt = ts;
  }
  w = next_w((size_t)D * Hd);
  if ((rc = launch_gemm(h_cur, w, rows, D, Hd, params[3 + 8 * blocks], no_stats, nullptr, none, 0, raw, none,
                        nullptr, stream)))
    return rc;
  return sslam_l2norm_rows(raw, rows, D, eps_norm, out_f32, out_bf16, out_hi, out_lo, stream_);
}

extern "C" void sslam_debug_gemm_stalls(long long* buf) { sslam::g_gemm_dbg = buf; }

extern "C" int sslam_refiner_range_check(void* stream_) {
  int rc = check_device();
  if (rc) return rc;
  cudaStream_t stream = (cudaStream_t)stream_;
  unsigned int h = 0;
  SSLAM_CHECK_CUDA(cudaMemcpyFromSymbolAsync(&h, sslam::g_refiner_status, sizeof(h), 0, cudaMemcpyDeviceToHost, stream));
  SSLAM_CHECK_CUDA(cudaStreamSynchronize(stream));
  if (h) {
    const unsigned int zero = 0;
    SSLAM_CHECK_CUDA(cudaMemcpyToSymbolAsync(sslam::g_refiner_status, &zero, sizeof(zero), 0, cudaMemcpyHostToDevice, stream));
    SSLAM_CHECK_CUDA(cudaStreamSynchronize(stream));
    SSLAM_REQUIRE(false, SSLAM_ERANGE,
                  "refiner: an activation reached the fp16 range (|x| >= 65504, or NaN / inf) in the f16x3 arithmetic");
  }
  return SSLAM_OK;
}

extern "C" void sslam_debug_refiner_fused(int mode) { sslam::g_refiner_fused = mode < 0 ? 0 : mode; }

extern "C" int sslam_debug_watchdog_gemm(unsigned long long* buf) {
  return (int)cudaMemcpyToSymbol(sslam::tc::g_watchdog_buf, &buf, sizeof(buf));
}
```

semantic-slam-master_b200/sslam_b200/_lib.py:

```python

import ctypes
import os

_HERE = os.path.dirname(os.path.abspath(__file__))
LIB_PATH = os.environ.get("SSLAM_B200_LIB") or os.path.join(_HERE, "libsslam_b200.so")

c_int, c_float, c_size_t, c_void_p = ctypes.c_int, ctypes.c_float, ctypes.c_size_t, ctypes.c_void_p

SIGNATURES = {
    "sslam_abi_version": (c_int, []),
    "sslam_last_error": (c_int, [ctypes.c_char_p, c_size_t]),
    "sslam_device_check": (c_int, []),
    "sslam_launch_count": (ctypes.c_uint64, []),
    "sslam_profile_enable": (c_int, [c_int]),
    "sslam_profile_kinds": (c_int, []),
    "sslam_profile_kind_name": (ctypes.c_char_p, [c_int]),
    "sslam_profile_read": (c_int, [c_int, ctypes.POINTER(ctypes.c_double), ctypes.POINTER(ctypes.c_uint64)]),
    "sslam_decode_workspace_bytes": (c_size_t, [c_int] * 4),
    "sslam_decode_topk_f32": (c_int, [c_void_p, c_int, c_int, c_int, c_int, c_int, c_int, c_float,
                                      c_float, c_void_p, c_void_p, c_void_p, c_void_p, c_size_t,
                                      c_void_p]),
    "sslam_nms_f32": (c_int, [c_void_p, c_int, c_int, c_int, c_int, c_void_p, c_void_p]),
    "sslam_gather_bilinear_f32": (c_int, [c_void_p, c_void_p, c_int, c_int, c_int, c_int, c_int,
                                          c_int, c_void_p, c_void_p, c_void_p, c_void_p]),
    "sslam_l2norm_rows": (c_int, [c_void_p, c_int, c_int, c_float, c_void_p, c_void_p, c_void_p, c_void_p,
                                  c_void_p]),
    "sslam_refiner_packed_bytes": (c_size_t, [c_int] * 4),
    "sslam_refiner_pack_weights": (c_int, [ctypes.POINTER(c_void_p), c_int, c_int, c_int, c_int, c_void_p,
                                           c_size_t, c_void_p]),
    "sslam_refiner_workspace_bytes": (c_size_t, [c_int] * 5),
    "sslam_refiner_forward_f32": (c_int, [ctypes.POINTER(c_void_p), c_void_p, c_void_p, c_void_p, c_void_p, c_int, c_int,
                                          c_int, c_int, c_int, c_float, c_void_p, c_void_p, c_void_p, c_void_p,
                                          c_void_p, c_size_t, c_void_p]),
    "sslam_refiner_range_check": (c_int, [c_void_p]),
    "sslam_match_workspace_bytes": (c_size_t, [c_int] * 7),
    "sslam_match_top2": (c_int, [c_void_p, c_void_p, c_int, c_void_p, c_void_p, c_int, c_void_p, c_int, c_int,
                                 c_int, c_int, c_int,
                                 c_void_p, c_void_p, c_void_p, c_void_p, c_void_p, c_void_p,
                                 c_size_t, c_void_p]),
    "sslam_match_finalize": (c_int, [c_int, ctypes.POINTER(ctypes.c_double), c_void_p, c_int, c_int, c_int,
                                     c_void_p, c_void_p, c_void_p, c_void_p, c_void_p, c_void_p,
                                     c_void_p, c_void_p, c_void_p, c_void_p, c_void_p, c_void_p,
                                     c_void_p]),
    "sslam_nn_points": (c_int, [c_void_p, c_int, c_void_p, c_int, c_void_p, c_void_p, c_int, c_int, c_int,
                                c_void_p, c_void_p, c_void_p]),
    "sslam_gt_matches": (c_int, [c_void_p, c_void_p, c_int, ctypes.c_double, c_int, c_int, c_void_p, c_void_p,
                                 c_void_p]),
    "sslam_eval_matches": (c_int, [c_void_p, c_void_p, c_int, c_void_p, c_void_p, c_int, c_int, c_int,
                                   c_void_p, c_void_p, c_void_p]),
    "sslam_selector_packed_bytes": (c_size_t, [c_int, c_int]),
    "sslam_selector_pack_weights": (c_int, [c_void_p, c_int, c_int, c_void_p, c_size_t, c_void_p]),
    "sslam_selector_workspace_bytes": (c_size_t, [c_int] * 4),
    "sslam_selector_head_f32": (c_int, [c_void_p, c_void_p, c_void_p, c_void_p, c_void_p, c_int, c_int, c_int,
                                        c_int, c_int, c_int, c_void_p, c_void_p, c_size_t, c_void_p]),
    "sslam_heatmap_from_cells_f32": (c_int, [c_void_p, c_int, c_int, c_int, c_int, c_int, c_void_p, c_void_p]),
    "sslam_ransac_workspace_bytes": (c_size_t, [c_int] * 3),
    "sslam_ransac_homography": (c_int, [c_void_p, c_int, c_void_p, c_int, c_void_p, c_int, c_int, c_int,
                                        c_void_p, c_void_p, c_void_p, c_int, c_int, ctypes.c_double, ctypes.c_uint64,
                                        c_void_p, c_void_p, c_void_p, c_void_p, c_void_p, c_void_p, c_size_t,
                                        c_void_p]),
}

DEBUG_SIGNATURES = {
    "sslam_debug_match_stalls": (None, [c_void_p]),
    "sslam_debug_gemm_stalls": (None, [c_void_p]),
    "sslam_debug_watchdog_gemm": (c_int, [c_void_p]),
    "sslam_debug_decode_stream": (None, [c_int]),
    "sslam_debug_refiner_fused": (None, [c_int]),
    "sslam_debug_decode_tune": (None, [c_int, c_int]),
}

ERROR_NAMES = {-1: "SSLAM_EINVAL", -2: "SSLAM_EUNSUPPORTED", -3: "SSLAM_EWORKSPACE",
               -4: "SSLAM_ECUDA", -5: "SSLAM_ENODEVICE", -6: "SSLAM_ERANGE"}

_lib = None
ABI_VERSION = 4


class SslamError(RuntimeError):
    def __init__(self, code, text):
        super().__init__(f"{ERROR_NAMES.get(code, code)}: {text}")
        self.code = code


def load():
    global _lib
    if _lib is None:
        if not os.path.exists(LIB_PATH):
            raise ImportError(
                f"{LIB_PATH} is missing: build it with `python -c 'import __graft_entry__ as g; "
                "g.build()'` or `make -C semantic-slam-master_b200/csrc`. There is no CPU fallback.")
        lib = ctypes.CDLL(LIB_PATH)
        for name, (res, args) in list(SIGNATURES.items()) + list(DEBUG_SIGNATURES.items()):
            fn = getattr(lib, name)
            fn.restype, fn.argtypes = res, args
        if lib.sslam_abi_version() != ABI_VERSION:
            raise ImportError("libsslam_b200.so ABI version mismatch; rebuild")
        _lib = lib
    return _lib


def last_error():
    buf = ctypes.create_string_buffer(512)
    load().sslam_last_error(buf, 512)
    return buf.value.decode(errors="replace")


def check(code):
    if code != 0:
        raise SslamError(code, last_error())
```

semantic-slam-master_b200/sslam_b200/ops.py:

```python

import ctypes

import torch

from . import _lib

SIM_F32, SIM_TF32X3, SIM_BF16, SIM_F16X3 = 0, 1, 2, 3
M1, M2, M3, M4, M5 = 1, 2, 3, 4, 5


def _stream():
    return ctypes.c_void_p(torch.cuda.current_stream().cuda_stream)


def _ptr(t):
    return ctypes.c_void_p(t.data_ptr()) if t is not None else ctypes.c_void_p(0)


def _need_cuda(*tensors):
    for t in tensors:
        if t is not None and not t.is_cuda:
            raise RuntimeError("sslam_b200 operates on CUDA tensors only (no CPU fallback)")


def launch_count():
    return int(_lib.load().sslam_launch_count())


def profile_enable(on=True):
    _lib.check(_lib.load().sslam_profile_enable(1 if on else 0))


def profile_read():
    lib = _lib.load()
    out = {}
    for k in range(lib.sslam_profile_kinds()):
        ms, n = ctypes.c_double(0), ctypes.c_uint64(0)
        _lib.check(lib.sslam_profile_read(k, ctypes.byref(ms), ctypes.byref(n)))
        if n.value:
            out[lib.sslam_profile_kind_name(k).decode()] = (ms.value, int(n.value))
    return out


class Workspace:

    def __init__(self):
        self.buf = None

    def get(self, nbytes, device):
        if self.buf is None or self.buf.numel() < nbytes or self.buf.device != device:
            self.buf = torch.empty(max(int(nbytes), 256), dtype=torch.uint8, device=device)
        return self.buf


_default_ws = {}


def _ws(kind, nbytes, device):
    key = (kind, device.index, torch.cuda.current_stream().cuda_stream)
    w = _default_ws.setdefault(key, Workspace())
    return w.get(nbytes, device)


def decode_topk(saliency, num_keypoints, nms_radius=2, min_score_percentile=0.5, floor=0.1,
                from_logits=False, out=None, workspace=None):
    lib = _lib.load()
    _need_cuda(saliency)
    sal = saliency[..., 0] if saliency.dim() == 4 else saliency
    if sal.dtype != torch.float32:
        raise RuntimeError("decode_topk expects fp32 saliency")
    sal = sal.contiguous()
    B, H, W = sal.shape
    K = int(num_keypoints)
    if out is None:
        kp = torch.empty(B, K, 2, dtype=torch.float32, device=sal.device)
        sc = torch.empty(B, K, dtype=torch.float32, device=sal.device)
        info = torch.empty(B, 4, dtype=torch.int32, device=sal.device)
    else:
        kp, sc, info = out
    need = lib.sslam_decode_workspace_bytes(B, H, W, K)
    ws = workspace if workspace is not None else _ws("decode", need, sal.device)
    _lib.check(lib.sslam_decode_topk_f32(_ptr(sal), int(bool(from_logits)), B, H, W, K,
                                         int(nms_radius), float(min_score_percentile), float(floor),
                                         _ptr(kp), _ptr(sc), _ptr(info), _ptr(ws), ws.numel(),
                                         _stream()))
    return kp, sc, info


def nms(saliency, radius):
    lib = _lib.load()
    _need_cuda(saliency)
    sal = saliency.contiguous()
    B, H, W = sal.shape
    out = torch.empty_like(sal)
    _lib.check(lib.sslam_nms_f32(_ptr(sal), B, H, W, int(radius), _ptr(out), _stream()))
    return out


def gather_bilinear(features, keypoints, pixel_coords=False, out=None, pair=False):
    lib = _lib.load()
    _need_cuda(features, keypoints)
    feat = features.contiguous()
    kp = keypoints.contiguous()
    if feat.dtype != torch.float32 or kp.dtype != torch.float32:
        raise RuntimeError("gather_bilinear expects fp32 tensors")
    B, h, w, C = feat.shape
    N = kp.shape[1]
    hi = lo = None
    if pair:
        hi = torch.empty(B, N, C, dtype=torch.float16, device=feat.device)
        lo = torch.empty(B, N, C, dtype=torch.float16, device=feat.device)
    elif out is None:
        out = torch.empty(B, N, C, dtype=torch.float32, device=feat.device)
    _lib.check(lib.sslam_gather_bilinear_f32(_ptr(feat), _ptr(kp), B, h, w, C, N,
                                             1 if pixel_coords else 0, _ptr(out), _ptr(hi), _ptr(lo),
                                             _stream()))
    return (hi, lo) if pair else out


def l2norm_rows(x, eps=1e-12, out=None, out_bf16=None, want_bf16=False, pair=None):
    lib = _lib.load()
    _need_cuda(x)
    xc = x.contiguous()
    D = xc.shape[-1]
    rows = xc.numel() // D
    if out is None:
        out = torch.empty_like(xc)
    if want_bf16 and out_bf16 is None:
        out_bf16 = torch.empty(xc.shape, dtype=torch.bfloat16, device=xc.device)
    hi, lo = _check_pair(pair, rows * D)
    _lib.check(lib.sslam_l2norm_rows(_ptr(xc), rows, D, float(eps), _ptr(out), _ptr(out_bf16), _ptr(hi),
                                     _ptr(lo), _stream()))
    return (out, out_bf16) if want_bf16 else out


def _check_pair(pair, numel):
    if pair is None:
        return None, None
    hi, lo = pair
    for t in (hi, lo):
        if t.dtype != torch.float16 or not t.is_contiguous() or t.numel() != numel:
            raise RuntimeError("fp16 pair outputs must be contiguous fp16 tensors of the result's size")
    return hi, lo


class RefinerPlan:

    def __init__(self, tensors, C, Hd, D, blocks):
        lib = _lib.load()
        _need_cuda(*tensors)
        self.tensors = [t.detach().contiguous() for t in tensors]
        for t in self.tensors:
            if t.dtype != torch.float32:
                raise RuntimeError("refiner parameters must be fp32")
        self.C, self.Hd, self.D, self.blocks = int(C), int(Hd), int(D), int(blocks)
        assert len(self.tensors) == 4 + 8 * self.blocks
        self.ptrs = (ctypes.c_void_p * len(self.tensors))(*[t.data_ptr() for t in self.tensors])
        dev = self.tensors[0].device
        nbytes = lib.sslam_refiner_packed_bytes(self.C, self.Hd, self.D, self.blocks)
        self.packed = torch.empty(nbytes, dtype=torch.uint8, device=dev)
        _lib.check(lib.sslam_refiner_pack_weights(self.ptrs, self.C, self.Hd, self.D, self.blocks,
                                                  _ptr(self.packed), nbytes, _stream()))


def refiner_forward(plan, x, eps=1e-12, want_bf16=False, workspace=None, out=None, out16=None, out_pair=None):
    lib = _lib.load()
    x_hi = x_lo = None
    if isinstance(x, (tuple, list)):
        x_hi, x_lo = (t.contiguous() for t in x)
        _need_cuda(x_hi, x_lo)
        if x_hi.dtype != torch.float16 or x_lo.dtype != torch.float16 or x_hi.shape[-1] != plan.C:
            raise RuntimeError("refiner_forward expects an fp16 (hi, lo) pair with %d channels" % plan.C)
        xc, rows = None, x_hi.numel() // plan.C
        ref = x_hi
    else:
        _need_cuda(x)
        xc = x.contiguous()
        if xc.dtype != torch.float32 or xc.shape[-1] != plan.C:
            raise RuntimeError("refiner_forward expects fp32 input with %d channels" % plan.C)
        rows = xc.numel() // plan.C
        ref = xc
    xc_dev = ref.device
    if out is None:
        out = torch.empty(rows, plan.D, dtype=torch.float32, device=xc_dev)
    if want_bf16 and out16 is None:
        out16 = torch.empty(rows, plan.D, dtype=torch.bfloat16, device=xc_dev)
    for t in (out, out16):
        if t is not None and (not t.is_contiguous() or t.numel() != rows * plan.D):
            raise RuntimeError("refiner_forward: output buffers must be contiguous (rows, D)")
    p_hi, p_lo = _check_pair(out_pair, rows * plan.D)
    need = lib.sslam_refiner_workspace_bytes(rows, plan.C, plan.Hd, plan.D, plan.blocks)
    ws = workspace if workspace is not None else _ws("refiner", need, xc_dev)
    _lib.check(lib.sslam_refiner_forward_f32(plan.ptrs, _ptr(plan.packed), _ptr(xc), _ptr(x_hi), _ptr(x_lo),
                                             rows, plan.C,
                                             plan.Hd, plan.D, plan.blocks, float(eps), _ptr(out),
                                             _ptr(out16), _ptr(p_hi), _ptr(p_lo), _ptr(ws), ws.numel(),
                                             _stream()))
    return (out, out16) if want_bf16 else out


def refiner_range_check():
    _lib.check(_lib.load().sslam_refiner_range_check(_stream()))


def match_top2(bank1, bank2, pair_index=None, mode=SIM_F16X3, num_pairs=None, workspace=None):
    lib = _lib.load()
    presplit = isinstance(bank1, (tuple, list))
    if presplit != isinstance(bank2, (tuple, list)):
        raise RuntimeError("either both descriptor banks are fp16 (hi, lo) pairs or neither")
    if presplit:
        if mode != SIM_F16X3:
            raise RuntimeError("fp16 (hi, lo) descriptor banks are the operand format of SIM_F16X3 only")
        (bank1, bank1_lo), (bank2, bank2_lo) = bank1, bank2
        _need_cuda(bank1, bank1_lo, bank2, bank2_lo)
        for t in (bank1, bank1_lo, bank2, bank2_lo):
            if t.dtype != torch.float16 or not t.is_contiguous():
                raise RuntimeError("fp16 (hi, lo) descriptor banks must be contiguous fp16")
        if bank1.shape != bank1_lo.shape or bank2.shape != bank2_lo.shape:
            raise RuntimeError("hi and lo halves of a descriptor bank must have the same shape")
    else:
        bank1_lo = bank2_lo = None
        _need_cuda(bank1, bank2, pair_index)
        if not (bank1.is_contiguous() and bank2.is_contiguous()):
            raise RuntimeError("descriptor banks must be contiguous")
        want = torch.bfloat16 if mode == SIM_BF16 else torch.float32
        if bank1.dtype != want or bank2.dtype != want:
            raise RuntimeError(f"mode {mode} expects {want} descriptor banks")
    N, D = bank1.shape[-2], bank1.shape[-1]
    M = bank2.shape[-2]
    if pair_index is not None:
        pair_index = pair_index.to(torch.int32).contiguous()
        P = pair_index.shape[0]
    else:
        P = int(num_pairs) if num_pairs is not None else min(bank1.shape[0], bank2.shape[0])
    dev = bank1.device
    res = dict(nn12=torch.empty(P, N, dtype=torch.int32, device=dev),
               best12=torch.empty(P, N, dtype=torch.float32, device=dev),
               second12=torch.empty(P, N, dtype=torch.float32, device=dev),
               nn21=torch.empty(P, M, dtype=torch.int32, device=dev),
               best21=torch.empty(P, M, dtype=torch.float32, device=dev))
    F1 = bank1.numel() // (N * D)
    F2 = bank2.numel() // (M * D)
    need = lib.sslam_match_workspace_bytes(F1, F2, P, N, M, D, mode)
    ws = workspace if workspace is not None else _ws("match", need, dev)
    _lib.check(lib.sslam_match_top2(_ptr(bank1), _ptr(bank1_lo), F1, _ptr(bank2), _ptr(bank2_lo), F2,
                                    _ptr(pair_index), int(mode), P, N, M,
                                    D, _ptr(res["nn12"]), _ptr(res["best12"]), _ptr(res["second12"]),
                                    _ptr(res["nn21"]), _ptr(res["best21"]), _ptr(ws), ws.numel(),
                                    _stream()))
    return res


def match_finalize(variant, top, params, pair_index=None, scores1=None, scores2=None,
                   inten1=None, inten2=None):
    lib = _lib.load()
    nn12 = top["nn12"]
    P, N = nn12.shape
    M = top["nn21"].shape[1]
    dev = nn12.device
    if pair_index is not None:
        pair_index = pair_index.to(torch.int32).contiguous()
    pairs = torch.empty(P, N, 2, dtype=torch.int32, device=dev)
    pscores = torch.empty(P, N, dtype=torch.float32, device=dev)
    counts = torch.empty(P, dtype=torch.int32, device=dev)
    prm = (ctypes.c_double * 8)(*([float(v) for v in params] + [0.0] * (8 - len(params))))
    for t in (scores1, scores2, inten1, inten2):
        if t is not None and (t.dtype != torch.float32 or not t.is_contiguous()):
            raise RuntimeError("score / intensity banks must be contiguous fp32")
    _lib.check(lib.sslam_match_finalize(int(variant), prm, _ptr(pair_index), P, N, M, _ptr(nn12),
                                        _ptr(top["best12"]), _ptr(top["second12"]), _ptr(top["nn21"]),
                                        _ptr(top["best21"]), _ptr(scores1), _ptr(scores2),
                                        _ptr(inten1), _ptr(inten2), _ptr(pairs), _ptr(pscores),
                                        _ptr(counts), _stream()))
    return pairs, pscores, counts


def nn_points(kpts1, kpts2, H=None, pair_index=None, num_pairs=None):
    lib = _lib.load()
    _need_cuda(kpts1, kpts2, H, pair_index)
    k1, k2 = kpts1.contiguous(), kpts2.contiguous()
    if k1.dtype != torch.float32 or k2.dtype != torch.float32:
        raise RuntimeError("nn_points expects fp32 keypoints")
    F1, N = k1.shape[0], k1.shape[1]
    F2, M = k2.shape[0], k2.shape[1]
    if pair_index is not None:
        pair_index = pair_index.to(torch.int32).contiguous()
        P = pair_index.shape[0]
    else:
        P = int(num_pairs) if num_pairs is not None else min(F1, F2)
    if H is not None:
        H = H.to(torch.float64).contiguous()
        if H.numel() != P * 9:
            raise RuntimeError("nn_points: H must hold one 3x3 matrix per pair")
    md = torch.empty(P, N, dtype=torch.float64 if H is not None else torch.float32, device=k1.device)
    am = torch.empty(P, N, dtype=torch.int32, device=k1.device)
    _lib.check(lib.sslam_nn_points(_ptr(k1), F1, _ptr(k2), F2, _ptr(H), _ptr(pair_index), P, N, M, _ptr(md),
                                   _ptr(am), _stream()))
    return md, am


def gt_matches(min_dist, argmin, threshold=3.0, want_pairs=True):
    lib = _lib.load()
    _need_cuda(min_dist, argmin)
    P, N = min_dist.shape
    md = min_dist.contiguous()
    pairs = torch.empty(P, N, 2, dtype=torch.int32, device=md.device) if want_pairs else None
    counts = torch.empty(P, dtype=torch.int32, device=md.device)
    _lib.check(lib.sslam_gt_matches(_ptr(md), _ptr(argmin.contiguous()), int(md.dtype == torch.float64),
                                    float(threshold), P, N, _ptr(pairs), _ptr(counts), _stream()))
    return pairs, counts


def eval_matches(pred_pairs, pred_counts, gt_pairs, gt_counts, num_kpts1):
    lib = _lib.load()
    _need_cuda(pred_pairs, pred_counts, gt_pairs, gt_counts)
    P = pred_pairs.shape[0]
    pp, gp = pred_pairs.to(torch.int32).contiguous(), gt_pairs.to(torch.int32).contiguous()
    scratch = torch.empty(P, int(num_kpts1), dtype=torch.int32, device=pp.device)
    out = torch.empty(P, 3, dtype=torch.int32, device=pp.device)
    _lib.check(lib.sslam_eval_matches(_ptr(pp), _ptr(pred_counts.to(torch.int32).contiguous()), pp.shape[1],
                                      _ptr(gp), _ptr(gt_counts.to(torch.int32).contiguous()), gp.shape[1], P,
                                      int(num_kpts1), _ptr(scratch), _ptr(out), _stream()))
    return out


def ransac_homography(kpts1, kpts2, pairs, pair_scores, counts, pair_index=None, num_pairs=None, threshold=3.0,
                      iters=1024, seed=0, want_mask=False, workspace=None):
    lib = _lib.load()
    _need_cuda(kpts1, kpts2, pairs, pair_scores, counts, pair_index)
    k1, k2 = kpts1.contiguous(), kpts2.contiguous()
    if k1.dtype != torch.float32 or k2.dtype != torch.float32:
        raise RuntimeError("ransac_homography expects fp32 keypoints")
    pr = pairs.to(torch.int32).contiguous()
    ps = pair_scores.to(torch.float32).contiguous()
    cn = counts.to(torch.int32).contiguous()
    F1, N = k1.shape[0], k1.shape[1]
    F2, M = k2.shape[0], k2.shape[1]
    P, L = pr.shape[0], pr.shape[1]
    if pair_index is not None:
        pair_index = pair_index.to(torch.int32).contiguous()
        if pair_index.shape[0] != P:
            raise RuntimeError("ransac_homography: pair_index must hold one (a, b) row per match list")
    elif num_pairs is not None and int(num_pairs) != P:
        raise RuntimeError("ransac_homography: num_pairs differs from the number of match lists")
    dev = pr.device
    H = torch.empty(P, 3, 3, dtype=torch.float64, device=dev)
    out_pairs = torch.empty(P, L, 2, dtype=torch.int32, device=dev)
    out_scores = torch.empty(P, L, dtype=torch.float32, device=dev)
    out_counts = torch.empty(P, dtype=torch.int32, device=dev)
    mask = torch.empty(P, L, dtype=torch.uint8, device=dev) if want_mask else None
    need = lib.sslam_ransac_workspace_bytes(P, L, int(iters))
    ws = workspace if workspace is not None else _ws("ransac", need, dev)
    _lib.check(lib.sslam_ransac_homography(_ptr(k1), F1, _ptr(k2), F2, _ptr(pair_index), P, N, M, _ptr(pr),
                                           _ptr(ps), _ptr(cn), L, int(iters), float(threshold),
                                           int(seed) & 0xFFFFFFFFFFFFFFFF, _ptr(H), _ptr(out_pairs),
                                           _ptr(out_scores), _ptr(out_counts), _ptr(mask), _ptr(ws), ws.numel(),
                                           _stream()))
    return (H, out_pairs, out_scores, out_counts) + ((mask,) if want_mask else ())


def ransac_workspace_views(workspace, P, L, iters):
    def up(x):
        return (x + 255) // 256 * 256
    o_best = up(P * iters * 4)
    o_mask = o_best + up(P * 4)
    w = workspace
    return (w[:P * iters * 4].view(torch.int32).reshape(P, iters),
            w[o_best:o_best + P * 4].view(torch.int32),
            w[o_mask:o_mask + P * L].reshape(P, L))


def heatmap_from_cells(logits, cell=8, border=0):
    lib = _lib.load()
    _need_cuda(logits)
    x = logits.contiguous()
    if x.dtype != torch.float32 or x.dim() != 4 or x.shape[1] != cell * cell + 1:
        raise RuntimeError("heatmap_from_cells expects fp32 (B, cell*cell+1, Hc, Wc) logits")
    B, _, Hc, Wc = x.shape
    heat = torch.empty(B, Hc * cell, Wc * cell, dtype=torch.float32, device=x.device)
    _lib.check(lib.sslam_heatmap_from_cells_f32(_ptr(x), B, Hc, Wc, int(cell), int(border), _ptr(heat), _stream()))
    return heat


class SelectorPlan:

    def __init__(self, conv1_weight, conv1_bias, conv2_weight, conv2_bias):
        lib = _lib.load()
        _need_cuda(conv1_weight, conv1_bias, conv2_weight, conv2_bias)
        w1 = conv1_weight.detach().contiguous()
        if w1.dtype != torch.float32 or w1.dim() != 4 or tuple(w1.shape[2:]) != (3, 3):
            raise RuntimeError("selector head expects an fp32 [hidden, C, 3, 3] convolution weight")
        self.hidden, self.C = int(w1.shape[0]), int(w1.shape[1])
        self.b1 = conv1_bias.detach().contiguous()
        self.w2 = conv2_weight.detach().reshape(-1).contiguous()
        self.b2 = conv2_bias.detach().reshape(-1).contiguous()
        if self.w2.numel() != self.hidden or self.b2.numel() != 1:
            raise RuntimeError("selector head expects a [1, hidden, 1, 1] second convolution")
        nbytes = lib.sslam_selector_packed_bytes(self.C, self.hidden)
        self.packed = torch.empty(nbytes, dtype=torch.uint8, device=w1.device)
        _lib.check(lib.sslam_selector_pack_weights(_ptr(w1), self.C, self.hidden, _ptr(self.packed), nbytes,
                                                   _stream()))


def selector_head(plan, features, apply_sigmoid=True, out=None, workspace=None):
    lib = _lib.load()
    _need_cuda(features)
    f = features.contiguous()
    if f.dtype != torch.float32 or f.dim() != 4 or f.shape[-1] != plan.C:
        raise RuntimeError("selector_head expects fp32 (B,H,W,%d) features" % plan.C)
    B, H, W, C = f.shape
    if out is None:
        out = torch.empty(B, H, W, dtype=torch.float32, device=f.device)
    need = lib.sslam_selector_workspace_bytes(B, H, W, C)
    ws = workspace if workspace is not None else _ws("selector", need, f.device)
    _lib.check(lib.sslam_selector_head_f32(_ptr(f), _ptr(plan.packed), _ptr(plan.b1), _ptr(plan.w2), _ptr(plan.b2),
                                           B, H, W, C, plan.hidden, 1 if apply_sigmoid else 0, _ptr(out), _ptr(ws),
                                           ws.numel(), _stream()))
    return out
```

semantic-slam-master_b200/sslam_b200/pipeline.py:

```python

import torch

from . import matchers, ops
from .ops import SIM_BF16, SIM_F32, SIM_F16X3


class FrontEnd:
    def __init__(self, refiner, num_keypoints=2048, nms_radius=2, min_score_percentile=0.5,
                 grid="pixel", sim_mode=SIM_F16X3, patch_size=16):
        self.refiner = refiner.eval()
        self.K, self.r, self.pct = int(num_keypoints), int(nms_radius), float(min_score_percentile)
        self.grid, self.sim_mode, self.patch = grid, sim_mode, patch_size

    def _mark(self, timers, name):
        if timers is not None:
            ev = torch.cuda.Event(enable_timing=True)
            ev.record()
            timers.append((name, ev))

    @torch.no_grad()
    def extract(self, saliency, features, timers=None, out=None):
        self._mark(timers, "begin")
        dec_out = (out["keypoints"], out["scores"], out["info"]) if out is not None else None
        kp, sc, info = ops.decode_topk(saliency, self.K, self.r, self.pct, out=dec_out)
        self._mark(timers, "decode")
        fused = getattr(self.refiner, "mlp", "torch") == "tcgen05"
        sampled = ops.gather_bilinear(features, kp, pixel_coords=(self.grid == "pixel"), pair=fused)
        self._mark(timers, "gather")
        B = kp.shape[0]
        res = dict(scores=sc, info=info)
        want16 = self.sim_mode == SIM_BF16
        o32 = out["descriptors"] if out is not None else None
        o16 = out.get("descriptors_bf16") if out is not None else None
        opair = None
        if self.sim_mode == SIM_F16X3:
            if out is not None:
                opair = (out["descriptors_hi"], out["descriptors_lo"])
            else:
                D = self.refiner.output_dim
                opair = tuple(torch.empty(B * self.K, D, dtype=torch.float16, device=kp.device) for _ in range(2))
        if fused:
            res_d = self.refiner.forward_fused(sampled, want_bf16=want16, out=o32, out16=o16,
                                               out_pair=opair)
            self._mark(timers, "refiner_mlp")
        else:
            raw = self.refiner.forward_unnormalized(sampled)
            self._mark(timers, "refiner_mlp")
            res_d = ops.l2norm_rows(raw, out=o32, out_bf16=o16, want_bf16=want16, pair=opair)
        d32, d16 = res_d if want16 else (res_d, None)
        if want16:
            res["descriptors_bf16"] = d16.reshape(B, self.K, -1)
        if opair is not None:
            res["descriptors_hi"] = opair[0].reshape(B, self.K, -1)
            res["descriptors_lo"] = opair[1].reshape(B, self.K, -1)
        self._mark(timers, "l2norm")
        res["descriptors"] = d32.reshape(B, self.K, -1)
        res["keypoints_pixel"] = kp if self.grid == "pixel" else kp * self.patch + self.patch / 2
        return res

    def bank(self, feats, start=0, stop=None):
        sl = slice(start, stop)
        if self.sim_mode == SIM_BF16:
            return feats["descriptors_bf16"][sl]
        if self.sim_mode == SIM_F16X3 and "descriptors_hi" in feats:
            return (feats["descriptors_hi"][sl], feats["descriptors_lo"][sl])
        return feats["descriptors"][sl]

    @staticmethod
    def _shift(bank, k=1):
        return tuple(t[k:] for t in bank) if isinstance(bank, tuple) else bank[k:]

    @torch.no_grad()
    def match_consecutive(self, feats, variant=matchers.M1, timers=None, **kw):
        bank = self.bank(feats)
        F = feats["descriptors"].shape[0]
        sc = feats["scores"]
        self._mark(timers, "begin")
        top = ops.match_top2(bank, self._shift(bank), mode=self.sim_mode, num_pairs=F - 1)
        self._mark(timers, "match_top2")
        out = matchers.match(bank, self._shift(bank), variant, num_pairs=F - 1, mode=self.sim_mode,
                             scores1=sc, scores2=sc[1:], top=top, **kw)[:3]
        self._mark(timers, "match_finalize")
        return out

    @torch.no_grad()
    def match_pairs(self, feats, pair_index, variant=matchers.M1, **kw):
        bank = self.bank(feats)
        sc = feats["scores"]
        return matchers.match(bank, bank, variant, pair_index=pair_index, mode=self.sim_mode,
                              scores1=sc, scores2=sc, **kw)[:3]

    @torch.no_grad()
    def run_sequence(self, saliency, features, variant=matchers.M1, chunk=256, timers=None, **kw):
        T = saliency.shape[0]
        feats = self._alloc_bank(T, saliency.device)
        for s in range(0, T, chunk):
            e = min(T, s + chunk)
            self.extract(saliency[s:e], features[s:e], timers=timers, out=self._bank_slice(feats, s, e))
        if self.grid != "pixel":
            feats["keypoints_pixel"] = feats["keypoints"] * self.patch + self.patch / 2
        pairs, pscores, counts = self.match_consecutive(feats, variant, timers=timers, **kw)
        return feats, pairs, pscores, counts

    def check_range(self):
        if getattr(self.refiner, "mlp", "torch") == "tcgen05":
            ops.refiner_range_check()

    @torch.no_grad()
    def run_pairs(self, saliency, features, pair_index, variant=matchers.M1, chunk=256, timers=None, **kw):
        T = saliency.shape[0]
        feats = self._alloc_bank(T, saliency.device)
        for s in range(0, T, chunk):
            e = min(T, s + chunk)
            self.extract(saliency[s:e], features[s:e], timers=timers, out=self._bank_slice(feats, s, e))
        if self.grid != "pixel":
            feats["keypoints_pixel"] = feats["keypoints"] * self.patch + self.patch / 2
        self._mark(timers, "begin")
        pairs, pscores, counts = self.match_pairs(feats, pair_index, variant, **kw)
        self._mark(timers, "match")
        return feats, pairs, pscores, counts

    @torch.no_grad()
    def capture(self, fn, *args, **kw):
        side = torch.cuda.Stream()
        side.wait_stream(torch.cuda.current_stream())
        with torch.cuda.stream(side):
            for _ in range(2):
                fn(*args, **kw)
        torch.cuda.current_stream().wait_stream(side)
        torch.cuda.synchronize()
        graph = torch.cuda.CUDAGraph()
        with torch.cuda.graph(graph):
            out = fn(*args, **kw)
        return graph.replay, out

    @torch.no_grad()
    def run_pairs_host(self, saliency_host, features_host, pair_index, variant=matchers.M1, chunk=64,
                       out_host=None, **kw):
        dev = torch.device("cuda", torch.cuda.current_device())
        T = saliency_host.shape[0]
        compute = torch.cuda.current_stream()
        st, copy = self._staging(saliency_host, features_host, chunk, dev)
        feats = self._alloc_bank(T, dev)
        copy.wait_stream(compute)
        for ci, s in enumerate(range(0, T, chunk)):
            e = min(T, s + chunk)
            b = ci & 1
            with torch.cuda.stream(copy):
                if ci >= 2:
                    copy.wait_event(st["free"][b])
                st["sal"][b][:e - s].copy_(saliency_host[s:e], non_blocking=True)
                st["feat"][b][:e - s].copy_(features_host[s:e], non_blocking=True)
                ready = torch.cuda.Event()
                ready.record(copy)
            compute.wait_event(ready)
            self.extract(st["sal"][b][:e - s], st["feat"][b][:e - s], out=self._bank_slice(feats, s, e))
            st["free"][b].record(compute)
        res = self.match_pairs(feats, pair_index, variant, **kw)
        P = pair_index.shape[0]
        if out_host is None:
            out_host = (torch.empty((P, self.K, 2), dtype=torch.int32, pin_memory=True),
                        torch.empty((P, self.K), dtype=torch.float32, pin_memory=True),
                        torch.empty((P,), dtype=torch.int32, pin_memory=True))
        for dst, src in zip(out_host, res):
            dst.copy_(src, non_blocking=True)
        compute.synchronize()
        self.check_range()
        return out_host

    def _staging(self, saliency_host, features_host, chunk, dev):
        if not hasattr(self, "_copy_stream"):
            self._copy_stream = torch.cuda.Stream()
            self._stage = {}
        key = (tuple(saliency_host.shape[1:]), tuple(features_host.shape[1:]), chunk)
        if self._stage.get("key") != key:
            self._stage = dict(key=key,
                               sal=[torch.empty((chunk,) + tuple(saliency_host.shape[1:]), device=dev) for _ in range(2)],
                               feat=[torch.empty((chunk,) + tuple(features_host.shape[1:]), device=dev) for _ in range(2)],
                               free=[torch.cuda.Event(), torch.cuda.Event()])
        return self._stage, self._copy_stream

    def _alloc_bank(self, T, device):
        D = self.refiner.output_dim
        bank = dict(keypoints=torch.empty(T, self.K, 2, device=device),
                    scores=torch.empty(T, self.K, device=device),
                    info=torch.empty(T, 4, dtype=torch.int32, device=device),
                    descriptors=torch.empty(T, self.K, D, device=device))
        if self.sim_mode == SIM_BF16:
            bank["descriptors_bf16"] = torch.empty(T, self.K, D, dtype=torch.bfloat16, device=device)
        if self.sim_mode == SIM_F16X3:
            bank["descriptors_hi"] = torch.empty(T, self.K, D, dtype=torch.float16, device=device)
            bank["descriptors_lo"] = torch.empty(T, self.K, D, dtype=torch.float16, device=device)
        bank["keypoints_pixel"] = bank["keypoints"]
        return bank

    def _bank_slice(self, bank, s, e):
        return {k: v[s:e] for k, v in bank.items() if k != "keypoints_pixel"}

    @torch.no_grad()
    def capture_sequence(self, saliency, features, variant=matchers.M1, chunk=256, **kw):
        side = torch.cuda.Stream()
        side.wait_stream(torch.cuda.current_stream())
        with torch.cuda.stream(side):
            for _ in range(2):
                self.run_sequence(saliency, features, variant, chunk=chunk, **kw)
        torch.cuda.current_stream().wait_stream(side)
        torch.cuda.synchronize()
        graph = torch.cuda.CUDAGraph()
        with torch.cuda.graph(graph):
            feats, pairs, pscores, counts = self.run_sequence(saliency, features, variant, chunk=chunk, **kw)
        return graph.replay, feats, pairs, pscores, counts

    @torch.no_grad()
    def run_sequence_host(self, saliency_host, features_host, variant=matchers.M1, chunk=64,
                          out_host=None, **kw):
        dev = torch.device("cuda", torch.cuda.current_device())
        T = saliency_host.shape[0]
        compute = torch.cuda.current_stream()
        st, copy = self._staging(saliency_host, features_host, chunk, dev)
        feats = self._alloc_bank(T, dev)
        if out_host is None:
            out_host = (torch.empty((T - 1, self.K, 2), dtype=torch.int32, pin_memory=True),
                        torch.empty((T - 1, self.K), dtype=torch.float32, pin_memory=True),
                        torch.empty((T - 1,), dtype=torch.int32, pin_memory=True))
        copy.wait_stream(compute)
        for ci, s in enumerate(range(0, T, chunk)):
            e = min(T, s + chunk)
            b = ci & 1
            with torch.cuda.stream(copy):
                if ci >= 2:
                    copy.wait_event(st["free"][b])
                st["sal"][b][:e - s].copy_(saliency_host[s:e], non_blocking=True)
                st["feat"][b][:e - s].copy_(features_host[s:e], non_blocking=True)
                ready = torch.cuda.Event()
                ready.record(copy)
            compute.wait_event(ready)
            self.extract(st["sal"][b][:e - s], st["feat"][b][:e - s], out=self._bank_slice(feats, s, e))
            st["free"][b].record(compute)
            p0 = max(s - 1, 0)
            if e - 1 > p0:
                bank = self.bank(feats, p0, e)
                sc = feats["scores"][p0:e]
                res = matchers.match(bank, self._shift(bank), variant, num_pairs=e - 1 - p0, mode=self.sim_mode,
                                     scores1=sc, scores2=sc[1:], **kw)[:3]
                for dst, src in zip(out_host, res):
                    dst[p0:e - 1].copy_(src, non_blocking=True)
        compute.synchronize()
        self.check_range()
        return out_host
```

Baseline: 53570.

## Pipeline sequence extraction and matching across streams with SM budgets

Adds a multi-stream schedule for run_sequence. Decode and gather of the next chunk run on a low-priority side stream, l2-norm is split into slices, and matching of finished slices runs on a high-priority match stream, all ordered by events. New _ex entry points let the match and gather kernels cap their grid to a given number of SMs so concurrent kernels can share the GPU, and a raw refiner entry point separates the normalization step. The aim is to hide serial stage boundaries and idle SMs, at the cost of scheduling complexity and possible contention between concurrent kernels.

```diff
diff --git a/include/sslam_b200.h b/include/sslam_b200.h
--- a/include/sslam_b200.h
+++ b/include/sslam_b200.h
@@ -65,6 +65,9 @@
 int sslam_gather_bilinear_f32(const float* feat, const float* kpts, int B, int h, int w, int C,
                               int N, int coords, float* out, void* out_hi, void* out_lo,
                               void* stream);
+int sslam_gather_bilinear_f32_ex(const float* feat, const float* kpts, int B, int h, int w, int C,
+                                 int N, int coords, float* out, void* out_hi, void* out_lo,
+                                 int max_sms, void* stream);
 
 int sslam_l2norm_rows(const float* in, int rows, int D, float eps, float* out_f32,
                       void* out_bf16, void* out_hi, void* out_lo, void* stream);
@@ -78,6 +81,9 @@
                               int rows, int C, int Hd, int D, int blocks, float eps_norm,
                               float* out_f32, void* out_bf16, void* out_hi, void* out_lo,
                               void* ws, size_t ws_bytes, void* stream);
+int sslam_refiner_forward_raw_f32(const float* const* params, const void* packed, const float* x,
+                                  const void* x_hi, const void* x_lo, int rows, int C, int Hd, int D,
+                                  int blocks, float* raw_out, void* ws, size_t ws_bytes, void* stream);
 int sslam_refiner_range_check(void* stream);
 
 size_t sslam_match_workspace_bytes(int F1, int F2, int P, int N, int M, int D, int dtype);
@@ -85,6 +91,10 @@
                      const void* bank2_lo, int F2, const int32_t* pair_index, int dtype,
                      int P, int N, int M, int D, int32_t* nn12, float* best12, float* second12,
                      int32_t* nn21, float* best21, void* ws, size_t ws_bytes, void* stream);
+int sslam_match_top2_ex(const void* bank1, const void* bank1_lo, int F1, const void* bank2,
+                        const void* bank2_lo, int F2, const int32_t* pair_index, int dtype,
+                        int P, int N, int M, int D, int32_t* nn12, float* best12, float* second12,
+                        int32_t* nn21, float* best21, void* ws, size_t ws_bytes, int max_sms, void* stream);
 
 int sslam_match_finalize(int variant, const double* params ,
                          const int32_t* pair_index, int P, int N, int M, const int32_t* nn12,
diff --git a/semantic-slam-master_b200/csrc/gather.cu b/semantic-slam-master_b200/csrc/gather.cu
--- a/semantic-slam-master_b200/csrc/gather.cu
+++ b/semantic-slam-master_b200/csrc/gather.cu
@@ -318,6 +318,12 @@
 extern "C" int sslam_gather_bilinear_f32(const float* feat, const float* kpts, int B, int h, int w,
                                          int C, int N, int coords, float* out, void* out_hi_, void* out_lo_,
                                          void* stream_) {
+  return sslam_gather_bilinear_f32_ex(feat, kpts, B, h, w, C, N, coords, out, out_hi_, out_lo_, 0, stream_);
+}
+
+extern "C" int sslam_gather_bilinear_f32_ex(const float* feat, const float* kpts, int B, int h, int w,
+                                            int C, int N, int coords, float* out, void* out_hi_, void* out_lo_,
+                                            int max_sms, void* stream_) {
   __half* out_hi = static_cast<__half*>(out_hi_);
   __half* out_lo = static_cast<__half*>(out_lo_);
   int rc = check_device();
@@ -325,6 +331,7 @@
   cudaStream_t stream = (cudaStream_t)stream_;
   SSLAM_REQUIRE(B >= 0 && h > 0 && w > 0 && C > 0 && N >= 0, SSLAM_EINVAL, "gather: bad size");
   SSLAM_REQUIRE(coords == 0 || coords == 1, SSLAM_EINVAL, "gather: coords must be 0 or 1");
+  SSLAM_REQUIRE(max_sms >= 0, SSLAM_EINVAL, "gather: max_sms must be >= 0 (0 = every SM)");
   if (B == 0 || N == 0) return SSLAM_OK;
   SSLAM_REQUIRE(feat && kpts && (out || (out_hi && out_lo)), SSLAM_EINVAL, "gather: null pointer");
   SSLAM_REQUIRE((out_hi == nullptr) == (out_lo == nullptr), SSLAM_EINVAL, "gather: pair outputs go together");
@@ -344,7 +351,8 @@
       SSLAM_CHECK_CUDA(cudaFuncSetAttribute(gather_band_kernel<false>, cudaFuncAttributeMaxDynamicSharedMemorySize,
                                             227 * 1024 - 256));
     }
-    int ngroups = (8 * num_sms() + B - 1) / B;
+    const int sms = max_sms > 0 && max_sms < num_sms() ? max_sms : num_sms();
+    int ngroups = (8 * sms + B - 1) / B;
     if (ngroups > (h + 1) / 3) ngroups = (h + 1) / 3;
     if (ngroups < 1) ngroups = 1;
     const int per = (h + 1 + ngroups - 1) / ngroups;
diff --git a/semantic-slam-master_b200/csrc/match_f32.cu b/semantic-slam-master_b200/csrc/match_f32.cu
--- a/semantic-slam-master_b200/csrc/match_f32.cu
+++ b/semantic-slam-master_b200/csrc/match_f32.cu
@@ -278,7 +278,7 @@
 int match_top2_tc(const void* bank1, const void* bank1_lo, int F1, const void* bank2, const void* bank2_lo,
                   int F2, const int32_t* pair_index,
                   int dtype, int P, int N, int M, int D, int32_t* nn12, float* best12, float* second12,
-                  u64* colkeys, void* ws_extra, size_t ws_extra_bytes, cudaStream_t stream);
+                  u64* colkeys, void* ws_extra, size_t ws_extra_bytes, int max_sms, cudaStream_t stream);
 size_t match_tc_extra_workspace(int P, int N, int M, int D, int dtype, int F1, int F2);
 
 }
@@ -297,9 +297,19 @@
                                 int dtype, int P, int N, int M, int D, int32_t* nn12, float* best12,
                                 float* second12, int32_t* nn21, float* best21, void* ws,
                                 size_t ws_bytes, void* stream_) {
+  return sslam_match_top2_ex(bank1, bank1_lo, F1, bank2, bank2_lo, F2, pair_index, dtype, P, N, M, D, nn12, best12,
+                             second12, nn21, best21, ws, ws_bytes, 0, stream_);
+}
+
+extern "C" int sslam_match_top2_ex(const void* bank1, const void* bank1_lo, int F1, const void* bank2,
+                                   const void* bank2_lo, int F2, const int32_t* pair_index,
+                                   int dtype, int P, int N, int M, int D, int32_t* nn12, float* best12,
+                                   float* second12, int32_t* nn21, float* best21, void* ws,
+                                   size_t ws_bytes, int max_sms, void* stream_) {
   int rc = check_device();
   if (rc) return rc;
   cudaStream_t stream = (cudaStream_t)stream_;
+  SSLAM_REQUIRE(max_sms >= 0, SSLAM_EINVAL, "match: max_sms must be >= 0 (0 = every SM)");
   SSLAM_REQUIRE(P >= 0 && N >= 0 && M >= 0 && D > 0, SSLAM_EINVAL, "match: bad size");
   if (P == 0 || N == 0) return SSLAM_OK;
   SSLAM_REQUIRE(M > 0, SSLAM_EINVAL, "match: M must be > 0 (argmax of an empty row)");
@@ -344,7 +354,7 @@
   } else {
     rc = match_top2_tc(bank1, bank1_lo, F1, bank2, bank2_lo, F2, pair_index, dtype, P, N, M, D, nn12, best12,
                        second12, colkeys,
-                       reinterpret_cast<char*>(ws) + colbytes, ws_bytes - colbytes, stream);
+                       reinterpret_cast<char*>(ws) + colbytes, ws_bytes - colbytes, max_sms, stream);
     if (rc) return rc;
   }
   const long long total = (long long)P * M;
diff --git a/semantic-slam-master_b200/csrc/match_tc.cu b/semantic-slam-master_b200/csrc/match_tc.cu
--- a/semantic-slam-master_b200/csrc/match_tc.cu
+++ b/semantic-slam-master_b200/csrc/match_tc.cu
@@ -677,7 +677,7 @@
 
 template <int MODE>
 static int launch_res(const CUtensorMap& a_hi, const CUtensorMap& a_lo, const CUtensorMap& b_hi,
-                      const CUtensorMap& b_lo, const TcParams& tp, cudaStream_t stream) {
+                      const CUtensorMap& b_lo, const TcParams& tp, int sms, cudaStream_t stream) {
   using L = RSmem<MODE>;
   static DeviceOnce once;
   if (once.first_use()) {
@@ -685,7 +685,8 @@
                                           L::TOTAL));
   }
   const int items = ((((tp.N + BM - 1) / BM) + 1) / 2) * tp.P;
-  const int pairs = items < num_sms() / 2 ? items : num_sms() / 2;
+  const int budget = sms / 2 > 1 ? sms / 2 : 1;
+  const int pairs = items < budget ? items : budget;
   const int grid = 2 * pairs;
   SSLAM_LAUNCH(KK_MATCH_TC, stream,
                match_res_kernel<MODE><<<grid, R_THREADS, L::TOTAL, stream>>>(a_hi, a_lo, b_hi, b_lo, tp));
@@ -695,7 +696,8 @@
 int match_top2_tc(const void* bank1, const void* bank1_lo, int F1, const void* bank2, const void* bank2_lo,
                   int F2, const int32_t* pair_index,
                   int dtype, int P, int N, int M, int D, int32_t* nn12, float* best12, float* second12,
-                  u64* colkeys, void* ws_extra, size_t ws_extra_bytes, cudaStream_t stream) {
+                  u64* colkeys, void* ws_extra, size_t ws_extra_bytes, int max_sms, cudaStream_t stream) {
+  const int sms = max_sms > 0 && max_sms < num_sms() ? max_sms : num_sms();
   TcParams tp;
   tp.dbg = g_match_dbg;
   tp.pair_index = pair_index; tp.P = P; tp.N = N; tp.M = M; tp.D = D;
@@ -707,7 +709,7 @@
     if ((rc = make_tensor_map_2d(&a_hi, bank1, (uint64_t)F1 * N, D, BM, 64, 2))) return rc;
     if ((rc = make_tensor_map_2d(&b_hi, bank2, (uint64_t)F2 * M, D, BN / 2, 64, 2))) return rc;
     a_lo = a_hi; b_lo = b_hi;
-    return launch_res<SSLAM_SIM_BF16>(a_hi, a_lo, b_hi, b_lo, tp, stream);
+    return launch_res<SSLAM_SIM_BF16>(a_hi, a_lo, b_hi, b_lo, tp, sms, stream);
   }
   const bool f16 = (dtype == SSLAM_SIM_F16X3);
   const size_t e = f16 ? 2 : 4;
@@ -718,7 +720,7 @@
     if ((rc = make_tensor_map_2d(&a_lo, bank1_lo, (uint64_t)F1 * N, D, BM, 64, 2))) return rc;
     if ((rc = make_tensor_map_2d(&b_hi, bank2, rows2p, D, BN / 2, 64, 2))) return rc;
     if ((rc = make_tensor_map_2d(&b_lo, bank2_lo, rows2p, D, BN / 2, 64, 2))) return rc;
-    return launch_res<SSLAM_SIM_F16X3>(a_hi, a_lo, b_hi, b_lo, tp, stream);
+    return launch_res<SSLAM_SIM_F16X3>(a_hi, a_lo, b_hi, b_lo, tp, sms, stream);
   }
   SSLAM_REQUIRE(ws_extra_bytes >= match_tc_extra_workspace(P, N, M, D, dtype, F1, F2), SSLAM_EWORKSPACE,
                 "match(split): workspace too small");
@@ -729,7 +731,6 @@
   const size_t n1 = pl.frames_a * (size_t)N * D;
   char* h1 = w;
   char* l1 = w + align_up(n1 * e, 256);
-  const int sms = num_sms();
   auto split = [&](const float* src, char* hi, char* lo, size_t n) -> int {
     if (f16)
       SSLAM_LAUNCH(KK_SPLIT, stream,
@@ -761,7 +762,7 @@
     if ((rc = make_tensor_map_2d(&a_lo, l1, (uint64_t)F1 * N, D, BM, 64, 2))) return rc;
     if ((rc = make_tensor_map_2d(&b_hi, h2, rows2, D, BN / 2, 64, 2))) return rc;
     if ((rc = make_tensor_map_2d(&b_lo, l2, rows2, D, BN / 2, 64, 2))) return rc;
-    return launch_res<SSLAM_SIM_F16X3>(a_hi, a_lo, b_hi, b_lo, tp, stream);
+    return launch_res<SSLAM_SIM_F16X3>(a_hi, a_lo, b_hi, b_lo, tp, sms, stream);
   }
   if ((rc = make_tensor_map_2d(&a_hi, h1, (uint64_t)F1 * N, D, BM, 32, 4))) return rc;
   if ((rc = make_tensor_map_2d(&a_lo, l1, (uint64_t)F1 * N, D, BM, 32, 4))) return rc;
diff --git a/semantic-slam-master_b200/csrc/refiner_tc.cu b/semantic-slam-master_b200/csrc/refiner_tc.cu
--- a/semantic-slam-master_b200/csrc/refiner_tc.cu
+++ b/semantic-slam-master_b200/csrc/refiner_tc.cu
@@ -1539,18 +1539,17 @@
          fused_scratch_bytes(rows, Hd);
 }
 
-extern "C" int sslam_refiner_forward_f32(const float* const* params, const void* packed, const float* x,
-                                         const void* x_hi, const void* x_lo,
-                                         int rows, int C, int Hd, int D, int blocks, float eps_norm,
-                                         float* out_f32, void* out_bf16, void* out_hi, void* out_lo,
-                                         void* ws, size_t ws_bytes, void* stream_) {
+static int refiner_forward(const float* const* params, const void* packed, const float* x, const void* x_hi,
+                           const void* x_lo, int rows, int C, int Hd, int D, int blocks, float eps_norm,
+                           float* out_f32, void* out_bf16, void* out_hi, void* out_lo, float* raw_out,
+                           void* ws, size_t ws_bytes, void* stream_) {
   int rc = check_device();
   if (rc) return rc;
   cudaStream_t stream = (cudaStream_t)stream_;
   SSLAM_REQUIRE(rows >= 0, SSLAM_EINVAL, "refiner: negative rows");
   if (rows == 0) return SSLAM_OK;
-  SSLAM_REQUIRE(params && packed && (x || (x_hi && x_lo)) && ws && (out_f32 || out_bf16 || out_hi), SSLAM_EINVAL,
-                "refiner: null pointer");
+  SSLAM_REQUIRE(params && packed && (x || (x_hi && x_lo)) && ws && (out_f32 || out_bf16 || out_hi || raw_out),
+                SSLAM_EINVAL, "refiner: null pointer");
   SSLAM_REQUIRE(C % 8 == 0 && Hd % 8 == 0 && D % 4 == 0 && Hd <= MAX_N && D <= MAX_N, SSLAM_EUNSUPPORTED,
                 "refiner: C and hidden must be multiples of 8, D of 4, hidden and D <= 1024 (C=%d Hd=%d D=%d)", C, Hd, D);
   SSLAM_REQUIRE(!x || (reinterpret_cast<uintptr_t>(x) & 15) == 0, SSLAM_EINVAL, "refiner: x must be 16-byte aligned");
@@ -1571,7 +1570,7 @@
   };
   Pair xs = take_pair(r * C), h_a = take_pair(r * Hd), h_b = take_pair(r * Hd), u = take_pair(r * Hd);
   RowStats st_a = take_stats(), st_b = take_stats(), st_u = take_stats();
-  float* raw = reinterpret_cast<float*>(wp);
+  float* raw = raw_out ? raw_out : reinterpret_cast<float*>(wp);
   char* fused_scratch = reinterpret_cast<char*>(align_up(reinterpret_cast<uintptr_t>(wp) + r * D * 4, 256));
   const char* pk = static_cast<const char*>(packed);
   auto next_w = [&](size_t n) {
@@ -1603,6 +1602,7 @@
       }
     layers[nl++] = FusedLayer{next_w((size_t)D * Hd), params[3 + 8 * blocks], nullptr};
     if ((rc = launch_fused(xs, layers, rows, C, Hd, D, blocks, raw, fused_scratch, stream))) return rc;
+    if (raw_out) return SSLAM_OK;
     return sslam_l2norm_rows(raw, rows, D, eps_norm, out_f32, out_bf16, out_hi, out_lo, stream_);
   }
   Pair w = next_w((size_t)Hd * C);
@@ -1632,7 +1632,27 @@
   if ((rc = launch_gemm(h_cur, w, rows, D, Hd, params[3 + 8 * blocks], no_stats, nullptr, none, 0, raw, none,
                         nullptr, stream)))
     return rc;
+  if (raw_out) return SSLAM_OK;
   return sslam_l2norm_rows(raw, rows, D, eps_norm, out_f32, out_bf16, out_hi, out_lo, stream_);
+}
+
+extern "C" int sslam_refiner_forward_f32(const float* const* params, const void* packed, const float* x,
+                                         const void* x_hi, const void* x_lo,
+                                         int rows, int C, int Hd, int D, int blocks, float eps_norm,
+                                         float* out_f32, void* out_bf16, void* out_hi, void* out_lo,
+                                         void* ws, size_t ws_bytes, void* stream_) {
+  return refiner_forward(params, packed, x, x_hi, x_lo, rows, C, Hd, D, blocks, eps_norm, out_f32, out_bf16,
+                         out_hi, out_lo, nullptr, ws, ws_bytes, stream_);
+}
+
+extern "C" int sslam_refiner_forward_raw_f32(const float* const* params, const void* packed, const float* x,
+                                             const void* x_hi, const void* x_lo, int rows, int C, int Hd, int D,
+                                             int blocks, float* raw_out, void* ws, size_t ws_bytes, void* stream_) {
+  SSLAM_REQUIRE(raw_out != nullptr || rows == 0, SSLAM_EINVAL, "refiner: null raw output");
+  SSLAM_REQUIRE((reinterpret_cast<uintptr_t>(raw_out) & 15) == 0, SSLAM_EINVAL,
+                "refiner: raw output must be 16-byte aligned");
+  return refiner_forward(params, packed, x, x_hi, x_lo, rows, C, Hd, D, blocks, 0.f, nullptr, nullptr, nullptr,
+                         nullptr, raw_out, ws, ws_bytes, stream_);
 }
 
 extern "C" void sslam_debug_gemm_stalls(long long* buf) { sslam::g_gemm_dbg = buf; }
diff --git a/semantic-slam-master_b200/sslam_b200/_lib.py b/semantic-slam-master_b200/sslam_b200/_lib.py
--- a/semantic-slam-master_b200/sslam_b200/_lib.py
+++ b/semantic-slam-master_b200/sslam_b200/_lib.py
@@ -23,6 +23,8 @@
     "sslam_nms_f32": (c_int, [c_void_p, c_int, c_int, c_int, c_int, c_void_p, c_void_p]),
     "sslam_gather_bilinear_f32": (c_int, [c_void_p, c_void_p, c_int, c_int, c_int, c_int, c_int,
                                           c_int, c_void_p, c_void_p, c_void_p, c_void_p]),
+    "sslam_gather_bilinear_f32_ex": (c_int, [c_void_p, c_void_p, c_int, c_int, c_int, c_int, c_int,
+                                             c_int, c_void_p, c_void_p, c_void_p, c_int, c_void_p]),
     "sslam_l2norm_rows": (c_int, [c_void_p, c_int, c_int, c_float, c_void_p, c_void_p, c_void_p, c_void_p,
                                   c_void_p]),
     "sslam_refiner_packed_bytes": (c_size_t, [c_int] * 4),
@@ -32,12 +34,19 @@
     "sslam_refiner_forward_f32": (c_int, [ctypes.POINTER(c_void_p), c_void_p, c_void_p, c_void_p, c_void_p, c_int, c_int,
                                           c_int, c_int, c_int, c_float, c_void_p, c_void_p, c_void_p, c_void_p,
                                           c_void_p, c_size_t, c_void_p]),
+    "sslam_refiner_forward_raw_f32": (c_int, [ctypes.POINTER(c_void_p), c_void_p, c_void_p, c_void_p, c_void_p,
+                                              c_int, c_int, c_int, c_int, c_int, c_void_p, c_void_p, c_size_t,
+                                              c_void_p]),
     "sslam_refiner_range_check": (c_int, [c_void_p]),
     "sslam_match_workspace_bytes": (c_size_t, [c_int] * 7),
     "sslam_match_top2": (c_int, [c_void_p, c_void_p, c_int, c_void_p, c_void_p, c_int, c_void_p, c_int, c_int,
                                  c_int, c_int, c_int,
                                  c_void_p, c_void_p, c_void_p, c_void_p, c_void_p, c_void_p,
                                  c_size_t, c_void_p]),
+    "sslam_match_top2_ex": (c_int, [c_void_p, c_void_p, c_int, c_void_p, c_void_p, c_int, c_void_p, c_int, c_int,
+                                    c_int, c_int, c_int,
+                                    c_void_p, c_void_p, c_void_p, c_void_p, c_void_p, c_void_p,
+                                    c_size_t, c_int, c_void_p]),
     "sslam_match_finalize": (c_int, [c_int, ctypes.POINTER(ctypes.c_double), c_void_p, c_int, c_int, c_int,
                                      c_void_p, c_void_p, c_void_p, c_void_p, c_void_p, c_void_p,
                                      c_void_p, c_void_p, c_void_p, c_void_p, c_void_p, c_void_p,
diff --git a/semantic-slam-master_b200/sslam_b200/ops.py b/semantic-slam-master_b200/sslam_b200/ops.py
--- a/semantic-slam-master_b200/sslam_b200/ops.py
+++ b/semantic-slam-master_b200/sslam_b200/ops.py
@@ -97,7 +97,7 @@
     return out
 
 
-def gather_bilinear(features, keypoints, pixel_coords=False, out=None, pair=False):
+def gather_bilinear(features, keypoints, pixel_coords=False, out=None, pair=False, max_sms=0, out_pair=None):
     lib = _lib.load()
     _need_cuda(features, keypoints)
     feat = features.contiguous()
@@ -107,14 +107,16 @@
     B, h, w, C = feat.shape
     N = kp.shape[1]
     hi = lo = None
-    if pair:
+    if pair and out_pair is not None:
+        hi, lo = _check_pair(out_pair, B * N * C)
+    elif pair:
         hi = torch.empty(B, N, C, dtype=torch.float16, device=feat.device)
         lo = torch.empty(B, N, C, dtype=torch.float16, device=feat.device)
     elif out is None:
         out = torch.empty(B, N, C, dtype=torch.float32, device=feat.device)
-    _lib.check(lib.sslam_gather_bilinear_f32(_ptr(feat), _ptr(kp), B, h, w, C, N,
-                                             1 if pixel_coords else 0, _ptr(out), _ptr(hi), _ptr(lo),
-                                             _stream()))
+    _lib.check(lib.sslam_gather_bilinear_f32_ex(_ptr(feat), _ptr(kp), B, h, w, C, N,
+                                                1 if pixel_coords else 0, _ptr(out), _ptr(hi), _ptr(lo),
+                                                int(max_sms), _stream()))
     return (hi, lo) if pair else out
 
 
@@ -199,11 +201,28 @@
     return (out, out16) if want_bf16 else out
 
 
+def refiner_forward_raw(plan, x, out, workspace=None):
+    lib = _lib.load()
+    x_hi, x_lo = (t.contiguous() for t in x)
+    _need_cuda(x_hi, x_lo, out)
+    if x_hi.dtype != torch.float16 or x_lo.dtype != torch.float16 or x_hi.shape[-1] != plan.C:
+        raise RuntimeError("refiner_forward_raw expects an fp16 (hi, lo) pair with %d channels" % plan.C)
+    rows = x_hi.numel() // plan.C
+    if out.dtype != torch.float32 or not out.is_contiguous() or out.numel() != rows * plan.D:
+        raise RuntimeError("refiner_forward_raw: out must be a contiguous fp32 (rows, D) tensor")
+    need = lib.sslam_refiner_workspace_bytes(rows, plan.C, plan.Hd, plan.D, plan.blocks)
+    ws = workspace if workspace is not None else _ws("refiner", need, x_hi.device)
+    _lib.check(lib.sslam_refiner_forward_raw_f32(plan.ptrs, _ptr(plan.packed), None, _ptr(x_hi), _ptr(x_lo), rows,
+                                                 plan.C, plan.Hd, plan.D, plan.blocks, _ptr(out), _ptr(ws),
+                                                 ws.numel(), _stream()))
+    return out
+
+
 def refiner_range_check():
     _lib.check(_lib.load().sslam_refiner_range_check(_stream()))
 
 
-def match_top2(bank1, bank2, pair_index=None, mode=SIM_F16X3, num_pairs=None, workspace=None):
+def match_top2(bank1, bank2, pair_index=None, mode=SIM_F16X3, num_pairs=None, workspace=None, max_sms=0, out=None):
     lib = _lib.load()
     presplit = isinstance(bank1, (tuple, list))
     if presplit != isinstance(bank2, (tuple, list)):
@@ -234,25 +253,32 @@
     else:
         P = int(num_pairs) if num_pairs is not None else min(bank1.shape[0], bank2.shape[0])
     dev = bank1.device
-    res = dict(nn12=torch.empty(P, N, dtype=torch.int32, device=dev),
-               best12=torch.empty(P, N, dtype=torch.float32, device=dev),
-               second12=torch.empty(P, N, dtype=torch.float32, device=dev),
-               nn21=torch.empty(P, M, dtype=torch.int32, device=dev),
-               best21=torch.empty(P, M, dtype=torch.float32, device=dev))
+    res = out if out is not None else alloc_top2(P, N, M, dev)
     F1 = bank1.numel() // (N * D)
     F2 = bank2.numel() // (M * D)
     need = lib.sslam_match_workspace_bytes(F1, F2, P, N, M, D, mode)
     ws = workspace if workspace is not None else _ws("match", need, dev)
-    _lib.check(lib.sslam_match_top2(_ptr(bank1), _ptr(bank1_lo), F1, _ptr(bank2), _ptr(bank2_lo), F2,
-                                    _ptr(pair_index), int(mode), P, N, M,
-                                    D, _ptr(res["nn12"]), _ptr(res["best12"]), _ptr(res["second12"]),
-                                    _ptr(res["nn21"]), _ptr(res["best21"]), _ptr(ws), ws.numel(),
-                                    _stream()))
+    for k, t in res.items():
+        if not t.is_contiguous() or t.shape[0] != P:
+            raise RuntimeError(f"match_top2: out[{k!r}] must be contiguous with {P} rows")
+    _lib.check(lib.sslam_match_top2_ex(_ptr(bank1), _ptr(bank1_lo), F1, _ptr(bank2), _ptr(bank2_lo), F2,
+                                       _ptr(pair_index), int(mode), P, N, M,
+                                       D, _ptr(res["nn12"]), _ptr(res["best12"]), _ptr(res["second12"]),
+                                       _ptr(res["nn21"]), _ptr(res["best21"]), _ptr(ws), ws.numel(),
+                                       int(max_sms), _stream()))
     return res
 
 
+def alloc_top2(P, N, M, device):
+    return dict(nn12=torch.empty(P, N, dtype=torch.int32, device=device),
+                best12=torch.empty(P, N, dtype=torch.float32, device=device),
+                second12=torch.empty(P, N, dtype=torch.float32, device=device),
+                nn21=torch.empty(P, M, dtype=torch.int32, device=device),
+                best21=torch.empty(P, M, dtype=torch.float32, device=device))
+
+
 def match_finalize(variant, top, params, pair_index=None, scores1=None, scores2=None,
-                   inten1=None, inten2=None):
+                   inten1=None, inten2=None, out=None):
     lib = _lib.load()
     nn12 = top["nn12"]
     P, N = nn12.shape
@@ -260,9 +286,14 @@
     dev = nn12.device
     if pair_index is not None:
         pair_index = pair_index.to(torch.int32).contiguous()
-    pairs = torch.empty(P, N, 2, dtype=torch.int32, device=dev)
-    pscores = torch.empty(P, N, dtype=torch.float32, device=dev)
-    counts = torch.empty(P, dtype=torch.int32, device=dev)
+    if out is not None:
+        pairs, pscores, counts = out
+        if not all(t.is_contiguous() and t.shape[0] == P for t in out):
+            raise RuntimeError(f"match_finalize: out tensors must be contiguous with {P} rows")
+    else:
+        pairs = torch.empty(P, N, 2, dtype=torch.int32, device=dev)
+        pscores = torch.empty(P, N, dtype=torch.float32, device=dev)
+        counts = torch.empty(P, dtype=torch.int32, device=dev)
     prm = (ctypes.c_double * 8)(*([float(v) for v in params] + [0.0] * (8 - len(params))))
     for t in (scores1, scores2, inten1, inten2):
         if t is not None and (t.dtype != torch.float32 or not t.is_contiguous()):
diff --git a/semantic-slam-master_b200/sslam_b200/pipeline.py b/semantic-slam-master_b200/sslam_b200/pipeline.py
--- a/semantic-slam-master_b200/sslam_b200/pipeline.py
+++ b/semantic-slam-master_b200/sslam_b200/pipeline.py
@@ -5,7 +5,52 @@
 from .ops import SIM_BF16, SIM_F32, SIM_F16X3
 
 
+def sequence_schedule(T, chunk, slices=4):
+    ops_ = []
+
+    def add(stream, op, lo, hi, after=(), budget=None):
+        ops_.append(dict(stream=stream, op=op, lo=lo, hi=hi, after=list(after)))
+        if budget is not None:
+            ops_[-1]["budget"] = budget
+        return len(ops_) - 1
+
+    def last(stream):
+        return max((i for i, o in enumerate(ops_) if o["stream"] == stream), default=None)
+
+    starts = list(range(0, T, chunk))
+    add("main", "D", 0, min(T, chunk))
+    add("main", "G", 0, min(T, chunk))
+    for ci, s in enumerate(starts):
+        e = min(T, s + chunk)
+        joins = [i for i in (last("side"), last("match")) if i is not None]
+        add("main", "R", s, e, joins)
+        n = max(1, min(slices, e - s))
+        bounds = [s + (e - s) * k // n for k in range(n + 1)]
+        first_n = add("main", "N", bounds[0], bounds[1])
+        side_n = {}
+        for k in range(1, n):
+            side_n[k] = add("side", "N", bounds[k], bounds[k + 1], [first_n] if k == 1 else [])
+        if ci + 1 < len(starts):
+            s2, e2 = starts[ci + 1], min(T, starts[ci + 1] + chunk)
+            add("side", "D", s2, e2, [first_n] if n == 1 else [])
+            add("side", "G", s2, e2)
+        more_side = ci + 1 < len(starts)
+        for k in range(n):
+            lo, hi = max(bounds[k] - 1, 0), bounds[k + 1] - 1
+            if hi <= lo:
+                continue
+            after = [first_n] if k == 0 else [side_n[k]]
+            add("match", "M", lo, hi, after, budget=more_side or k + 1 < n)
+    joins = [i for i in (last("side"), last("match")) if i is not None]
+    add("main", "join", T, T, joins)
+    return ops_
+
+
 class FrontEnd:
+    pipeline = True
+    match_sms = 116
+    match_slices = 4
+
     def __init__(self, refiner, num_keypoints=2048, nms_radius=2, min_score_percentile=0.5,
                  grid="pixel", sim_mode=SIM_F16X3, patch_size=16):
         self.refiner = refiner.eval()
@@ -91,8 +136,13 @@
                               scores1=sc, scores2=sc, **kw)[:3]
 
     @torch.no_grad()
-    def run_sequence(self, saliency, features, variant=matchers.M1, chunk=256, timers=None, **kw):
+    def run_sequence(self, saliency, features, variant=matchers.M1, chunk=256, timers=None, pipelined=None, **kw):
         T = saliency.shape[0]
+        if pipelined is None:
+            pipelined = (self.pipeline and timers is None and self.sim_mode == SIM_F16X3
+                         and getattr(self.refiner, "mlp", "torch") == "tcgen05")
+        if pipelined:
+            return self._run_sequence_pipelined(saliency, features, variant, chunk, **kw)
         feats = self._alloc_bank(T, saliency.device)
         for s in range(0, T, chunk):
             e = min(T, s + chunk)
@@ -101,6 +151,71 @@
             feats["keypoints_pixel"] = feats["keypoints"] * self.patch + self.patch / 2
         pairs, pscores, counts = self.match_consecutive(feats, variant, timers=timers, **kw)
         return feats, pairs, pscores, counts
+
+    def _run_sequence_pipelined(self, saliency, features, variant, chunk, **kw):
+        T = saliency.shape[0]
+        dev = saliency.device
+        D, C = self.refiner.output_dim, features.shape[-1]
+        main = torch.cuda.current_stream()
+        if getattr(self, "_streams", None) is None or self._streams[0].device != dev:
+            lo_prio, hi_prio = torch.cuda.Stream.priority_range()
+            self._streams = (torch.cuda.Stream(device=dev, priority=hi_prio),
+                             torch.cuda.Stream(device=dev, priority=lo_prio))
+        streams = dict(main=main, match=self._streams[0], side=self._streams[1])
+        feats = self._alloc_bank(T, dev)
+        n0 = min(T, chunk)
+        sampled = tuple(torch.empty(n0 * self.K * C, dtype=torch.float16, device=dev) for _ in range(2))
+        raw = torch.empty(n0 * self.K, D, dtype=torch.float32, device=dev)
+        P = T - 1
+        top = ops.alloc_top2(P, self.K, self.K, dev)
+        lists = (torch.empty(P, self.K, 2, dtype=torch.int32, device=dev),
+                 torch.empty(P, self.K, dtype=torch.float32, device=dev),
+                 torch.empty(P, dtype=torch.int32, device=dev))
+        bank = self.bank(feats)
+        sc = feats["scores"]
+        d32 = feats["descriptors"].reshape(T * self.K, D)
+        dhi = feats["descriptors_hi"].reshape(T * self.K, D)
+        dlo = feats["descriptors_lo"].reshape(T * self.K, D)
+        params = matchers.variant_params(variant, **kw)
+        sched = sequence_schedule(T, chunk, self.match_slices)
+        waited = {i for o in sched for i in o["after"]}
+        events = {}
+        chunk_lo = 0
+        for i, o in enumerate(sched):
+            st = streams[o["stream"]]
+            for j in o["after"]:
+                st.wait_event(events[j])
+            lo, hi = o["lo"], o["hi"]
+            n = hi - lo
+            with torch.cuda.stream(st):
+                if o["op"] == "D":
+                    ops.decode_topk(saliency[lo:hi], self.K, self.r, self.pct,
+                                    out=(feats["keypoints"][lo:hi], sc[lo:hi], feats["info"][lo:hi]))
+                elif o["op"] == "G":
+                    ops.gather_bilinear(features[lo:hi], feats["keypoints"][lo:hi], pixel_coords=(self.grid == "pixel"),
+                                        pair=True, out_pair=tuple(t[:n * self.K * C] for t in sampled))
+                elif o["op"] == "R":
+                    chunk_lo = lo
+                    ops.refiner_forward_raw(self.refiner._plan(),
+                                            tuple(t[:n * self.K * C].view(n * self.K, C) for t in sampled),
+                                            raw[:n * self.K])
+                elif o["op"] == "N":
+                    r0, r1 = (lo - chunk_lo) * self.K, (hi - chunk_lo) * self.K
+                    ops.l2norm_rows(raw[r0:r1], out=d32[lo * self.K:hi * self.K],
+                                    pair=(dhi[lo * self.K:hi * self.K], dlo[lo * self.K:hi * self.K]))
+                elif o["op"] == "M":
+                    part = tuple(t[lo:hi + 1] for t in bank)
+                    sl = {k: v[lo:hi] for k, v in top.items()}
+                    ops.match_top2(part, self._shift(part), mode=self.sim_mode, num_pairs=n,
+                                   max_sms=self.match_sms if o["budget"] else 0, out=sl)
+                    ops.match_finalize(variant, sl, params, scores1=sc[lo:hi + 1], scores2=sc[lo + 1:hi + 1],
+                                       out=tuple(t[lo:hi] for t in lists))
+            if i in waited:
+                events[i] = torch.cuda.Event()
+                events[i].record(st)
+        if self.grid != "pixel":
+            feats["keypoints_pixel"] = feats["keypoints"] * self.patch + self.patch / 2
+        return (feats,) + lists
 
     def check_range(self):
         if getattr(self.refiner, "mlp", "torch") == "tcgen05":
```

Result: slower. 52110, median of 6 (-2.7%).
